# sailor-z/3DAHV

Measured on AMD Instinct MI355X. Metric: rotation hypotheses scored/sec (B=1), higher is better.
Workload: dtype f32; 1 GPU; CO3D pair (BASELINE.json configs[1]): B=1, ONE set of N_hyp=50000 Haar rotations split over the GPUs (contiguous shards, n_offset), source volume 16x8x8x8 (P=512 voxel sites x 16 ch), head 384->32->32, 64 positions; n_hyp_per_gpu=50000, n_hyp_total=50000, parallelism=hypothesis axis sharded x1, 8-byte key all-reduce(max), backend=single process, lanes=1

## Files before the change

### 3dahv_amd/_lib.py

```python
from __future__ import annotations

import ctypes
import os
import subprocess

_HERE = os.path.dirname(os.path.abspath(__file__))
CSRC = os.path.join(_HERE, "csrc")
LIB_PATH = os.path.join(CSRC, "libahv_hip.so")

AHV_SCORE_RESET_BEST = 1
AHV_SCORE_SPLIT_F16 = 2
AHV_SCORE_NO_TEAMS = 4
AHV_SCORE_SPARE_CUS_SHIFT = 8
AHV_SELECT_RESET_KEY = 1
AHV_KEY_EMPTY = -(1 << 63)
AHV_TOPK_MAX_K = 64
AHV_TOPK_RESET_LIST = 1
AHV_SO3_MAX_LADDER = 8
AHV_POSTERIOR_MAX_MODES = 16
AHV_POSTERIOR_RESET_STATE = 1
AHV_VIEWS_MAX = 16
AHV_VIEWS_RESET_BEST = 1
AHV_VIEWS_NO_ANGLE_LIMIT = 2

_vp = ctypes.c_void_p
_i64 = ctypes.c_int64
_int = ctypes.c_int
_u32 = ctypes.c_uint

SIGNATURES = {
    "ahv_abi_version": (_int, []),
    "ahv_last_error": (ctypes.c_char_p, []),
    "ahv_device_cu_count": (_int, []),
    "ahv_score_hypotheses_f32": (_int, [_vp, _vp, _vp, _i64, _i64, _vp, _vp, _vp, _int, _i64, _vp, _vp, _u32, _vp]),
    "ahv_score_hypotheses_clocked_f32": (_int, [_vp, _vp, _vp, _i64, _i64, _vp, _vp, _vp, _int, _i64, _vp, _vp, _u32,
                                                _vp, _vp]),
    "ahv_verify_pair_f32": (_int, [_vp, _vp, _vp, _i64, _i64, _vp, _vp, _vp, _int, _i64, _vp, _vp, _vp, _u32, _vp, _vp]),
    "ahv_unpack_best": (_int, [_vp, _int, _vp, _vp, _vp]),
    "ahv_reset_best": (_int, [_vp, _int, _vp]),
    "ahv_rotate_volume_f32": (_int, [_vp, _i64, _vp, _i64, _int, _int, _int, _int, _vp, _vp]),
    "ahv_rotate_volume_backward_f32": (_int, [_vp, _i64, _vp, _i64, _int, _int, _int, _int, _vp, _vp]),
    "ahv_forward_3d2d_f32": (_int, [_vp, _vp, _vp, _vp, _i64, _vp, _vp]),
    "ahv_score_features_f32": (_int, [_vp, _vp, _int, _i64, _vp, _vp]),
    "ahv_argmax_f32": (_int, [_vp, _int, _i64, _i64, _vp, _u32, _vp]),
    "ahv_random_rotations_f32": (_int, [ctypes.c_uint64, ctypes.c_uint64, _i64, _vp, _vp]),
    "ahv_so3_grid_f32": (_int, [_i64, _i64, _i64, _vp, _vp]),
    "ahv_select_rotation_f32": (_int, [_vp, _vp, _i64, _i64, _i64, _int, _vp, _vp, _vp, _u32, _vp]),
    "ahv_compose_rotations_f32": (_int, [_vp, _vp, _i64, _i64, _i64, _vp, _i64, _int, _vp, _vp]),
    "ahv_coarse_to_fine_f32": (_int, [_vp, _vp, _vp, _i64, _i64, _vp, _i64, _vp, _vp, _vp, _int, _vp, _vp, _vp, _vp, _vp,
                                      _vp, _vp, _vp, _vp, _vp, _u32, _vp]),
}

class BlockWeights(ctypes.Structure):
    _fields_ = [(n, _vp) for n in ("w_qkv", "w_out", "b_out", "ln1_g", "ln1_b", "w_ff1", "b_ff1", "w_ff2", "b_ff2",
                                   "ln2_g", "ln2_b")]


class AlignerWeights(ctypes.Structure):
    _fields_ = ([(n, _vp) for n in ("w_emb", "w_conv1", "w_conv2", "posemb", "gn_g", "gn_b")] +
                [("w_in", _vp * 2), ("b_in", _vp * 2), ("w_out", _vp * 2), ("b_out", _vp * 2),
                 ("w3d_1", _vp), ("w3d_2", _vp), ("blocks", ctypes.POINTER(BlockWeights)), ("depth", _int)])


SIGNATURES["ahv_forward_2d3d_workspace_bytes"] = (ctypes.c_size_t, [_int])
SIGNATURES["ahv_forward_2d3d_f32"] = (_int, [ctypes.POINTER(AlignerWeights), _vp, _vp, _int, _vp, ctypes.c_size_t, _vp,
                                             _vp, _vp])
SIGNATURES["ahv_score_hypotheses_backward_workspace_bytes"] = (ctypes.c_size_t, [_int, _i64])
SIGNATURES["ahv_score_hypotheses_backward_f32"] = (_int, [_vp, _vp, _vp, _i64, _vp, _vp, _vp, _int, _i64, _vp, _vp,
                                                          ctypes.c_size_t, _vp, _vp, _vp, _vp, _vp, _vp])
SIGNATURES["ahv_score_hypotheses_backward_saved_f32"] = SIGNATURES["ahv_score_hypotheses_backward_f32"]
SIGNATURES["ahv_score_hypotheses_train_f32"] = (_int, [_vp, _vp, _vp, _i64, _vp, _vp, _vp, _int, _i64, _vp, _vp, ctypes.c_size_t, _vp])
SIGNATURES["ahv_transformer_workspace_bytes"] = (ctypes.c_size_t, [_int])
SIGNATURES["ahv_transformer_blocks_f32"] = (_int, [ctypes.POINTER(BlockWeights), _int, _vp, _vp, _int, _vp,
                                                   ctypes.c_size_t, _vp])
SIGNATURES["ahv_topk_workspace_bytes"] = (ctypes.c_size_t, [_int, _i64, _int])
SIGNATURES["ahv_topk_f32"] = (_int, [_vp, _int, _i64, _i64, _int, _vp, _vp, ctypes.c_size_t, _u32, _vp])
SIGNATURES["ahv_topk_merge_keys"] = (_int, [_vp, _int, _int, _int, _vp, _u32, _vp])
SIGNATURES["ahv_select_topk_f32"] = (_int, [_vp, _int, _vp, _i64, _i64, _i64, _int, _vp, _vp, _vp, _u32, _vp])
SIGNATURES["ahv_compose_rotations_topk_f32"] = (_int, [_vp, _int, _vp, _i64, _i64, _i64, _vp, _i64, _int, _vp, _vp])
SIGNATURES["ahv_topk_modes_workspace_bytes"] = (ctypes.c_size_t, [_int, _i64, _int])
SIGNATURES["ahv_topk_modes_f32"] = (_int, [_vp, _vp, _i64, _int, _i64, _i64, _int, ctypes.c_float, _vp, _vp, ctypes.c_size_t, _vp])
SIGNATURES["ahv_score_rotation_grad_workspace_bytes"] = (ctypes.c_size_t, [_int, _i64])
SIGNATURES["ahv_score_rotation_grad_f32"] = (_int, [_vp, _vp, _vp, _i64, _vp, _vp, _vp, _int, _i64, _vp, _vp, ctypes.c_size_t,
                                                    _vp, _vp])
SIGNATURES["ahv_so3_ascent_candidates_f32"] = (_int, [_vp, _vp, _vp, _vp, _int, _int, _int, _vp, _vp])
SIGNATURES["ahv_so3_ascent_select_f32"] = (_int, [_vp, _vp, _vp, _int, _int, _int, _vp, _vp, _vp, _vp])
SIGNATURES["ahv_pose_posterior_state_bytes"] = (ctypes.c_size_t, [_int, _int])
SIGNATURES["ahv_pose_posterior_workspace_bytes"] = (ctypes.c_size_t, [_int, _i64, _int])
SIGNATURES["ahv_pose_posterior_f32"] = (_int, [_vp, _vp, _i64, _int, _i64, _vp, _int, ctypes.c_float, ctypes.c_float, _vp, _vp,
                                               ctypes.c_size_t, _u32, _vp])
SIGNATURES["ahv_pose_posterior_merge"] = (_int, [_vp, _int, _int, _int, ctypes.c_float, _vp, _u32, _vp])
SIGNATURES["ahv_pose_posterior_finish_f32"] = (_int, [_vp, _int, _int, ctypes.c_float] + [_vp] * 10 + [_vp])
SIGNATURES["ahv_view_rotations_f32"] = (_int, [_vp, _i64, _vp, _int, _int, _i64, _vp, _vp])
SIGNATURES["ahv_fuse_view_scores_f32"] = (_int, [_vp, _vp, _i64, _vp, _vp, _int, _int, _i64, _i64, ctypes.c_float, _vp, _vp, _u32,
                                                 _vp])

DIAG_SIGNATURES = {
    "ahv_score_hypotheses_clocked_f32": SIGNATURES.pop("ahv_score_hypotheses_clocked_f32"),
    "ahv_diag_score_plan": (_int, [_int, _i64, _u32, ctypes.POINTER(_int), ctypes.POINTER(_int), ctypes.POINTER(_i64)]),
}

_lib = None


class AhvError(RuntimeError):
    """A libahv_hip call returned a negative status."""


def build(force: bool = False) -> str:
    args = ["make", "-C", CSRC, "-j4"] + (["-B"] if force else [])
    proc = subprocess.run(args, stdout=subprocess.PIPE, stderr=subprocess.STDOUT, text=True)
    if proc.returncode != 0:
        raise RuntimeError("building libahv_hip.so failed:\n" + proc.stdout)
    return LIB_PATH


def load():
    global _lib
    if _lib is not None:
        return _lib
    import torch
    if not os.path.exists(LIB_PATH):
        raise ImportError(
            f"{LIB_PATH} not found: the HIP extension is required (no CPU fallback). "
            "Run `python -c 'import __graft_entry__ as g; g.build()'` or `make -C 3dahv_amd/csrc`."
        )
    lib = ctypes.CDLL(LIB_PATH)
    for name, (res, args) in list(SIGNATURES.items()) + list(DIAG_SIGNATURES.items()):
        fn = getattr(lib, name)
        fn.restype = res
        fn.argtypes = args
    _lib = lib
    return lib


def check(status: int, what: str) -> None:
    if status < 0:
        msg = load().ahv_last_error().decode("utf-8", "replace")
        raise AhvError(f"{what} failed with status {status}: {msg}")
```

### 3dahv_amd/csrc/ahv_abi.hip

```cpp
#include <hip/hip_runtime.h>

#include <cstdarg>
#include <cstdio>
#include <cstring>

#include "../../include/ahv.h"
#include "../../include/ahv_diag.h"
#include "ahv_launch.h"

namespace ahv {
hipError_t launch_unpack_best(const int64_t*, int, float*, int64_t*, hipStream_t);
hipError_t launch_rotate_volume(const float*, int64_t, const float*, int64_t, int, int, int, int, float*, int,
                                hipStream_t);
hipError_t launch_rotate_volume_backward(const float*, int64_t, const float*, int64_t, int, int, int, int, float*, int,
                                         hipStream_t);
hipError_t launch_forward_3d2d(const float*, const float*, const float*, const float*, int64_t, float*, int,
                               hipStream_t);
hipError_t launch_score_features(const float*, const float*, int, int64_t, float*, int, hipStream_t);
hipError_t launch_argmax(const float*, int, int64_t, int64_t, int64_t*, int, hipStream_t);
hipError_t launch_fill_keys(int64_t*, int, hipStream_t);
int topk_parts(int64_t N);
hipError_t launch_topk(const float*, int, int64_t, int64_t, int, int64_t*, int64_t*, bool, hipStream_t);
hipError_t launch_topk_merge(const int64_t*, int, int, int, int64_t*, bool, hipStream_t);
hipError_t launch_select_topk(int64_t*, int, const float*, int64_t, int64_t, int64_t, int, float*, float*, int64_t*, bool,
                              hipStream_t);
hipError_t launch_compose_rotations_topk(const int64_t*, int, const float*, int64_t, int64_t, int64_t, const float*, int64_t,
                                         int, float*, hipStream_t);
int64_t topk_modes_state_stride(int64_t N);
hipError_t launch_topk_modes(const float*, const float*, int64_t, int, int64_t, int64_t, int, float, int64_t*, int64_t*,
                             hipStream_t);
hipError_t launch_view_rotations(const float*, int64_t, const float*, int, int, int64_t, float*, hipStream_t);
hipError_t launch_fuse_views(const float*, const float*, int64_t, const float*, const float*, int, int, int64_t, int64_t, float,
                             bool, float*, int64_t*, hipStream_t);
size_t posterior_state_stride(int K);
int posterior_parts(int64_t N);
hipError_t launch_posterior(const float*, const float*, int64_t, int, int64_t, const float*, int, float, float, void*, void*, bool,
                            hipStream_t);
hipError_t launch_posterior_merge(const void*, int, int, int, float, void*, bool, hipStream_t);
hipError_t launch_posterior_finish(const void*, int, int, float, float*, float*, float*, int64_t*, float*, float*, float*, float*,
                                   float*, float*, hipStream_t);
hipError_t launch_random_rotations(uint64_t, uint64_t, int64_t, float*, hipStream_t);
hipError_t launch_so3_grid(int64_t, int64_t, int64_t, float*, hipStream_t);
hipError_t launch_score_backward(const float*, const float*, const float*, int64_t, const float*, const float*,
                                 const float*, int, int64_t, const float*, float*, float*, float*, float*, float*,
                                 float*, float*, int, hipStream_t, bool);
hipError_t launch_zero_fill(void* const* ptrs, const size_t* bytes, int count, hipStream_t stream);
hipError_t launch_score_rotation_grad(const float*, const float*, const float*, int64_t, const float*, const float*,
                                      const float*, int, int64_t, const float*, float*, float*, int, hipStream_t);
hipError_t launch_so3_ascent_candidates(const float*, const float*, const float*, const float*, int, int, int, float*,
                                        hipStream_t);
hipError_t launch_so3_ascent_select(const float*, const float*, const float*, int, int, int, float*, float*, float*,
                                    hipStream_t);
size_t transformer_workspace_floats(int B);
int transformer_blocks(const ahv_block_weights*, int, float*, float*, int, float*, hipStream_t, const char**);
size_t forward_2d3d_workspace_floats(int B);
int forward_2d3d(const ahv_aligner_weights*, const float*, const float*, int, float*, float*, float*, hipStream_t,
                 const char**);
}

namespace {

thread_local char g_err[256] = "";

int fail(int code, const char* fmt, ...)
{
    va_list ap;
    va_start(ap, fmt);
    vsnprintf(g_err, sizeof(g_err), fmt, ap);
    va_end(ap);
    return code;
}

int hip_fail(const char* what, hipError_t e)
{
    return fail(AHV_ELAUNCH, "%s: %s", what, hipGetErrorString(e));
}

int cu_count()
{
    static thread_local int cached_dev = -1, cached_cu = 0;
    int dev = 0;
    if (hipGetDevice(&dev) != hipSuccess) return -1;
    if (dev != cached_dev) {
        int cu = 0;
        if (hipDeviceGetAttribute(&cu, hipDeviceAttributeMultiprocessorCount, dev) != hipSuccess || cu <= 0)
            return -1;
        cached_dev = dev;
        cached_cu = cu;
    }
    return cached_cu;
}

}

extern "C" {

int ahv_abi_version(void) { return (2 << 16) | 3; }

const char* ahv_last_error(void) { return g_err; }

int ahv_device_cu_count(void)
{
    const int cu = cu_count();
    if (cu < 0) return fail(AHV_EDEVICE, "no usable HIP device");
    return cu;
}

static hipError_t zero_span(void* p, size_t bytes, hipStream_t s)
{
    void* const ptrs[1] = {p};
    const size_t n[1] = {bytes};
    return ahv::launch_zero_fill(ptrs, n, 1, s);
}

static int score_common(const char* who, const float* vol_src, const float* tgt, bool tgt_is_volume, const float* R,
                        int64_t r_batch_stride, int64_t n_offset, const float* W1, const float* W2, const float* b2, int B,
                        int64_t N, float* scores, int64_t* best_key, float* feat_tgt_out, unsigned flags,
                        uint64_t* clock_stamps, void* stream)
{
    if (B < 0 || N < 0) return fail(AHV_EINVAL, "%s: negative size (B=%d, N=%lld)", who, B, (long long)N);
    if (B > 0 && N > 0 && (!vol_src || !tgt || !R || !W1 || !W2 || !b2))
        return fail(AHV_EINVAL, "%s: null input pointer", who);
    if (r_batch_stride != 0 && r_batch_stride < N * 9)
        return fail(AHV_EINVAL, "%s: r_batch_stride %lld must be 0 or >= N*9", who, (long long)r_batch_stride);
    if (n_offset < 0 || n_offset + N > 4294967296ll)
        return fail(AHV_EINVAL, "%s: n_offset + N must fit in 32 bits", who);
    if (flags & ~(AHV_SCORE_RESET_BEST | AHV_SCORE_SPLIT_F16 | AHV_SCORE_NO_TEAMS | AHV_SCORE_SPARE_CUS_MASK))
        return fail(AHV_EINVAL, "%s: unknown flags 0x%x", who, flags);
    const bool split = (flags & AHV_SCORE_SPLIT_F16) != 0;
    hipStream_t s = static_cast<hipStream_t>(stream);
    if (best_key && (flags & AHV_SCORE_RESET_BEST) && B > 0) {
        hipError_t e = ahv::launch_fill_keys(best_key, B, s);
        if (e != hipSuccess) return hip_fail("score: key reset", e);
    }
    const int cu = cu_count();
    if (cu < 0) return fail(AHV_EDEVICE, "no usable HIP device");
    if (tgt_is_volume && split) {
        if (B > 0 && !feat_tgt_out)
            return fail(AHV_EINVAL, "%s: AHV_SCORE_SPLIT_F16 needs feat_tgt_out (the target features go through it)", who);
        if (B > 0) {
            hipError_t e = ahv::launch_forward_3d2d(tgt, W1, W2, b2, B, feat_tgt_out, cu, s);
            if (e != hipSuccess) return hip_fail("verify_pair: forward_3d2d launch", e);
        }
        tgt = feat_tgt_out;
        tgt_is_volume = false;
        feat_tgt_out = nullptr;
    }
    if (B == 0) return AHV_OK;
    if (N == 0 && !(tgt_is_volume && feat_tgt_out)) return AHV_OK;
    ahv::ScoreLaunch a;
    a.vol_src = vol_src; a.tgt = tgt; a.tgt_is_volume = tgt_is_volume; a.R = R;
    a.r_batch_stride = r_batch_stride; a.n_offset = n_offset; a.W1 = W1; a.W2 = W2; a.b2 = b2; a.B = B; a.N = N;
    a.scores = scores; a.best_key = best_key; a.feat_tgt_out = feat_tgt_out; a.num_cu = cu;
    a.spare_cu = (int)((flags & AHV_SCORE_SPARE_CUS_MASK) >> AHV_SCORE_SPARE_CUS_SHIFT);
    a.split_f16 = split; a.no_teams = (flags & AHV_SCORE_NO_TEAMS) != 0; a.clock_stamps = clock_stamps;
    hipError_t e = ahv::launch_score_hypotheses(a, s);
    if (e != hipSuccess) return hip_fail("score: launch", e);
    return AHV_OK;
}

int ahv_score_hypotheses_f32(const float* vol_src, const float* feat_tgt, const float* R,
                             int64_t r_batch_stride, int64_t n_offset, const float* W1, const float* W2,
                             const float* b2, int B, int64_t N, float* scores, int64_t* best_key,
                             unsigned flags, void* stream)
{
    return score_common("score", vol_src, feat_tgt, false, R, r_batch_stride, n_offset, W1, W2, b2, B, N, scores, best_key,
                        nullptr, flags, nullptr, stream);
}

int ahv_score_hypotheses_clocked_f32(const float* vol_src, const float* feat_tgt, const float* R,
                                     int64_t r_batch_stride, int64_t n_offset, const float* W1, const float* W2,
                                     const float* b2, int B, int64_t N, float* scores, int64_t* best_key,
                                     unsigned flags, uint64_t* clock_stamps, void* stream)
{
    if (!clock_stamps) return fail(AHV_EINVAL, "score_clocked: null clock_stamps");
    return score_common("score_clocked", vol_src, feat_tgt, false, R, r_batch_stride, n_offset, W1, W2, b2, B, N, scores,
                        best_key, nullptr, flags, clock_stamps, stream);
}

int ahv_diag_score_plan(int B, int64_t N, unsigned flags, int* gx, int* gy, int64_t* n_main)
{
    if (B < 1 || N < 0) return fail(AHV_EINVAL, "score_plan: bad shape (B=%d, N=%lld)", B, (long long)N);
    const int cu = cu_count();
    if (cu < 0) return fail(AHV_EDEVICE, "no usable HIP device");
    const bool teams = !(flags & AHV_SCORE_SPLIT_F16) && !(flags & AHV_SCORE_NO_TEAMS);
    const ahv::ScorePlan p = ahv::plan_score_launch(B, N, cu, (int)((flags & AHV_SCORE_SPARE_CUS_MASK) >> AHV_SCORE_SPARE_CUS_SHIFT), teams);
    if (gx) *gx = p.gx;
    if (gy) *gy = p.gy;
    if (n_main) *n_main = p.n_main;
    return AHV_OK;
}

int ahv_verify_pair_f32(const float* vol_src, const float* vol_tgt, const float* R, int64_t r_batch_stride,
                        int64_t n_offset, const float* W1, const float* W2, const float* b2, int B, int64_t N,
                        float* scores, int64_t* best_key, float* feat_tgt_out, unsigned flags, uint64_t* clock_stamps,
                        void* stream)
{
    return score_common("verify_pair", vol_src, vol_tgt, true, R, r_batch_stride, n_offset, W1, W2, b2, B, N, scores,
                        best_key, feat_tgt_out, flags, clock_stamps, stream);
}

int ahv_unpack_best(const int64_t* best_key, int B, float* best_score, int64_t* best_idx, void* stream)
{
    if (!best_key) return fail(AHV_EINVAL, "unpack: null best_key");
    if (B < 0) return fail(AHV_EINVAL, "unpack: negative B");
    if (B == 0) return AHV_OK;
    hipError_t e = ahv::launch_unpack_best(best_key, B, best_score, best_idx, static_cast<hipStream_t>(stream));
    if (e != hipSuccess) return hip_fail("unpack: launch", e);
    return AHV_OK;
}

int ahv_rotate_volume_f32(const float* vol, int64_t vol_batch_stride, const float* R, int64_t N, int C, int D,
                          int H, int W, float* out, void* stream)
{
    if (N < 0 || C < 1 || D < 1 || H < 1 || W < 1)
        return fail(AHV_EINVAL, "rotate_volume: bad shape N=%lld C=%d D=%d H=%d W=%d", (long long)N, C, D, H, W);
    if (vol_batch_stride < 0) return fail(AHV_EINVAL, "rotate_volume: negative batch stride");
    if (N == 0) return AHV_OK;
    if (!vol || !R || !out) return fail(AHV_EINVAL, "rotate_volume: null pointer");
    const int cu = cu_count();
    if (cu < 0) return fail(AHV_EDEVICE, "no usable HIP device");
    hipError_t e = ahv::launch_rotate_volume(vol, vol_batch_stride, R, N, C, D, H, W, out, cu,
                                             static_cast<hipStream_t>(stream));
    if (e != hipSuccess) return hip_fail("rotate_volume: launch", e);
    return AHV_OK;
}

int ahv_rotate_volume_backward_f32(const float* grad_out, int64_t vol_batch_stride, const float* R, int64_t N, int C,
                                   int D, int H, int W, float* grad_vol, void* stream)
{
    if (N < 0 || C < 1 || D < 1 || H < 1 || W < 1)
        return fail(AHV_EINVAL, "rotate_volume_backward: bad shape N=%lld C=%d D=%d H=%d W=%d", (long long)N, C, D, H, W);
    const int64_t vol_elems = (int64_t)C * D * H * W;
    if (vol_batch_stride != 0 && vol_batch_stride < vol_elems)
        return fail(AHV_EINVAL, "rotate_volume_backward: batch stride must be 0 or >= C*D*H*W");
    if (!grad_vol) return fail(AHV_EINVAL, "rotate_volume_backward: null grad_vol");
    hipStream_t s = static_cast<hipStream_t>(stream);
    const int64_t n_vol = vol_batch_stride == 0 ? 1 : N;
    if (n_vol > 0) {
        const size_t bytes = sizeof(float) * (size_t)(vol_batch_stride == 0 ? vol_elems : (N - 1) * vol_batch_stride + vol_elems);
        hipError_t e = zero_span(grad_vol, bytes, s);
        if (e != hipSuccess) return hip_fail("rotate_volume_backward: zero fill", e);
    }
    if (N == 0) return AHV_OK;
    if (!grad_out || !R) return fail(AHV_EINVAL, "rotate_volume_backward: null pointer");
    const int cu = cu_count();
    if (cu < 0) return fail(AHV_EDEVICE, "no usable HIP device");
    hipError_t e = ahv::launch_rotate_volume_backward(grad_out, vol_batch_stride, R, N, C, D, H, W, grad_vol, cu, s);
    if (e != hipSuccess) return hip_fail("rotate_volume_backward: launch", e);
    return AHV_OK;
}

int ahv_forward_3d2d_f32(const float* vol, const float* W1, const float* W2, const float* b2, int64_t M,
                         float* out, void* stream)
{
    if (M < 0) return fail(AHV_EINVAL, "forward_3d2d: negative M");
    if (M == 0) return AHV_OK;
    if (!vol || !W1 || !W2 || !b2 || !out) return fail(AHV_EINVAL, "forward_3d2d: null pointer");
    const int cu = cu_count();
    if (cu < 0) return fail(AHV_EDEVICE, "no usable HIP device");
    hipError_t e = ahv::launch_forward_3d2d(vol, W1, W2, b2, M, out, cu, static_cast<hipStream_t>(stream));
    if (e != hipSuccess) return hip_fail("forward_3d2d: launch", e);
    return AHV_OK;
}

int ahv_score_features_f32(const float* f_src, const float* f_tgt, int B, int64_t N, float* scores, void* stream)
{
    if (B < 0 || N < 0) return fail(AHV_EINVAL, "score_features: negative size");
    if (B == 0 || N == 0) return AHV_OK;
    if (!f_src || !f_tgt || !scores) return fail(AHV_EINVAL, "score_features: null pointer");
    const int cu = cu_count();
    if (cu < 0) return fail(AHV_EDEVICE, "no usable HIP device");
    hipError_t e = ahv::launch_score_features(f_src, f_tgt, B, N, scores, cu, static_cast<hipStream_t>(stream));
    if (e != hipSuccess) return hip_fail("score_features: launch", e);
    return AHV_OK;
}

int ahv_compose_rotations_f32(const int64_t* best_key, const float* R, int64_t r_batch_stride, int64_t n_offset,
                                 int64_t N, const float* D, int64_t N2, int B, float* out, void* stream)
{
    if (B < 0 || N < 0 || N2 < 0) return fail(AHV_EINVAL, "compose_rotations: negative size");
    if (B == 0 || N2 == 0) return AHV_OK;
    if (!best_key || !R || !D || !out) return fail(AHV_EINVAL, "compose_rotations: null pointer");
    if (N == 0) return fail(AHV_EINVAL, "compose_rotations: empty rotation set");
    if (r_batch_stride != 0 && r_batch_stride < N * 9) return fail(AHV_EINVAL, "compose_rotations: bad r_batch_stride");
    hipError_t e = ahv::launch_compose_rotations_topk(best_key, 1, R, r_batch_stride, n_offset, N, D, N2, B, out,
                                                      static_cast<hipStream_t>(stream));
    if (e != hipSuccess) return hip_fail("compose_rotations: launch", e);
    return AHV_OK;
}

int ahv_coarse_to_fine_f32(const float* vol_src, const float* vol_tgt, const float* R, int64_t r_batch_stride, int64_t N,
                           const float* D, int64_t N2, const float* W1, const float* W2, const float* b2, int B,
                           float* scores_coarse, float* scores_fine, int64_t* keys, uint32_t* sync, float* feat_tgt_out,
                           float* R_pred, float* fine_score, int64_t* fine_idx, float* coarse_score, int64_t* coarse_idx,
                           unsigned flags, void* stream)
{
    if (B < 0 || N < 0 || N2 < 0) return fail(AHV_EINVAL, "coarse_to_fine: negative size (B=%d, N=%lld, N2=%lld)", B, (long long)N, (long long)N2);
    if (B == 0) return AHV_OK;
    if (N == 0 || N2 == 0) return fail(AHV_EINVAL, "coarse_to_fine: empty hypothesis set (N=%lld, N2=%lld)", (long long)N, (long long)N2);
    if (!vol_src || !vol_tgt || !R || !D || !W1 || !W2 || !b2) return fail(AHV_EINVAL, "coarse_to_fine: null input pointer");
    if (!keys || !sync) return fail(AHV_EINVAL, "coarse_to_fine: keys and sync are required (2 B keys, 2 B + 1 counters)");
    if (r_batch_stride != 0 && r_batch_stride < N * 9)
        return fail(AHV_EINVAL, "coarse_to_fine: r_batch_stride %lld must be 0 or >= N*9", (long long)r_batch_stride);
    if (N > 4294967296ll || N2 > 4294967296ll) return fail(AHV_EINVAL, "coarse_to_fine: indices must fit in 32 bits");
    if (flags & ~(AHV_SCORE_NO_TEAMS | AHV_SCORE_SPARE_CUS_MASK)) return fail(AHV_EINVAL, "coarse_to_fine: unknown flags 0x%x", flags);
    const int cu = cu_count();
    if (cu < 0) return fail(AHV_EDEVICE, "no usable HIP device");
    ahv::CoarseToFineLaunch a;
    ahv::ScoreLaunch& c = a.coarse;
    c.vol_src = vol_src; c.tgt = vol_tgt; c.tgt_is_volume = true; c.R = R; c.r_batch_stride = r_batch_stride; c.n_offset = 0;
    c.W1 = W1; c.W2 = W2; c.b2 = b2; c.B = B; c.N = N; c.scores = scores_coarse; c.best_key = keys;
    c.feat_tgt_out = feat_tgt_out; c.num_cu = cu;
    c.spare_cu = (int)((flags & AHV_SCORE_SPARE_CUS_MASK) >> AHV_SCORE_SPARE_CUS_SHIFT);
    c.split_f16 = false; c.no_teams = (flags & AHV_SCORE_NO_TEAMS) != 0; c.clock_stamps = nullptr;
    a.D = D; a.N2 = N2; a.scores2 = scores_fine; a.best_key2 = keys + B; a.sync = sync; a.R_pred = R_pred;
    a.fine_score = fine_score; a.coarse_score = coarse_score; a.fine_idx = fine_idx; a.coarse_idx = coarse_idx;
    hipError_t e = ahv::launch_coarse_to_fine(a, static_cast<hipStream_t>(stream));
    if (e != hipSuccess) return hip_fail("coarse_to_fine: launch", e);
    return AHV_OK;
}

int ahv_reset_best(int64_t* best_key, int B, void* stream)
{
    if (B < 0) return fail(AHV_EINVAL, "reset_best: negative B");
    if (B == 0) return AHV_OK;
    if (!best_key) return fail(AHV_EINVAL, "reset_best: null best_key");
    hipError_t e = ahv::launch_fill_keys(best_key, B, static_cast<hipStream_t>(stream));
    if (e != hipSuccess) return hip_fail("reset_best: launch", e);
    return AHV_OK;
}

int ahv_select_rotation_f32(int64_t* best_key, const float* R, int64_t r_batch_stride, int64_t n_offset, int64_t N,
                            int B, float* R_out, float* best_score, int64_t* best_idx, unsigned flags, void* stream)
{
    if (B < 0 || N < 0) return fail(AHV_EINVAL, "select_rotation: negative size");
    if (flags & ~AHV_SELECT_RESET_KEY) return fail(AHV_EINVAL, "select_rotation: unknown flags 0x%x", flags);
    if (B == 0) return AHV_OK;
    if (!best_key) return fail(AHV_EINVAL, "select_rotation: null best_key");
    if (R_out && (!R || N == 0)) return fail(AHV_EINVAL, "select_rotation: R_out needs a rotation set");
    if (r_batch_stride != 0 && r_batch_stride < N * 9) return fail(AHV_EINVAL, "select_rotation: bad r_batch_stride");
    hipError_t e = ahv::launch_select_topk(best_key, 1, R, r_batch_stride, n_offset, N, B, R_out, best_score, best_idx,
                                           (flags & AHV_SELECT_RESET_KEY) != 0, static_cast<hipStream_t>(stream));
    if (e != hipSuccess) return hip_fail("select_rotation: launch", e);
    return AHV_OK;
}

size_t ahv_transformer_workspace_bytes(int B) { return sizeof(float) * ahv::transformer_workspace_floats(B); }

int ahv_transformer_blocks_f32(const ahv_block_weights* blocks, int depth, float* x_src, float* x_tgt, int B,
                               void* workspace, size_t workspace_bytes, void* stream)
{
    if (depth < 0 || B < 0) return fail(AHV_EINVAL, "transformer_blocks: negative size");
    if (depth == 0 || B == 0) return AHV_OK;
    if (!blocks || !x_src || !x_tgt || !workspace) return fail(AHV_EINVAL, "transformer_blocks: null pointer");
    if (workspace_bytes < ahv_transformer_workspace_bytes(B))
        return fail(AHV_EINVAL, "transformer_blocks: workspace of %zu bytes, need %zu", workspace_bytes,
                    ahv_transformer_workspace_bytes(B));
    if ((reinterpret_cast<uintptr_t>(workspace) & 15) || (reinterpret_cast<uintptr_t>(x_src) & 15) ||
        (reinterpret_cast<uintptr_t>(x_tgt) & 15))
        return fail(AHV_EINVAL, "transformer_blocks: buffers must be 16-byte aligned");
    for (int i = 0; i < 4 * depth; ++i) {
        const ahv_block_weights& w = blocks[i];
        if (!w.w_qkv || !w.w_out || !w.b_out || !w.ln1_g || !w.ln1_b || !w.w_ff1 || !w.b_ff1 || !w.w_ff2 || !w.b_ff2 ||
            !w.ln2_g || !w.ln2_b)
            return fail(AHV_EINVAL, "transformer_blocks: null weight pointer in block %d", i);
    }
    const char* what = "";
    const int rc = ahv::transformer_blocks(blocks, depth, x_src, x_tgt, B, static_cast<float*>(workspace),
                                           static_cast<hipStream_t>(stream), &what);
    if (rc != 0) return fail(AHV_ELAUNCH, "transformer_blocks: %s: %s", what, hipGetErrorString((hipError_t)rc));
    return AHV_OK;
}

size_t ahv_forward_2d3d_workspace_bytes(int B) { return sizeof(float) * ahv::forward_2d3d_workspace_floats(B); }

int ahv_forward_2d3d_f32(const ahv_aligner_weights* w, const float* layer4_src, const float* layer4_tgt, int B,
                         void* workspace, size_t workspace_bytes, float* vol_src, float* vol_tgt, void* stream)
{
    if (B < 0) return fail(AHV_EINVAL, "forward_2d3d: negative B");
    if (B == 0) return AHV_OK;
    if (!w || !layer4_src || !layer4_tgt || !workspace || !vol_src || !vol_tgt)
        return fail(AHV_EINVAL, "forward_2d3d: null pointer");
    if (!w->w_emb || !w->w_conv1 || !w->w_conv2 || !w->posemb || !w->gn_g || !w->gn_b || !w->w_in[0] || !w->w_in[1] ||
        !w->b_in[0] || !w->b_in[1] || !w->w_out[0] || !w->w_out[1] || !w->b_out[0] || !w->b_out[1] || !w->w3d_1 ||
        !w->w3d_2 || (w->depth > 0 && !w->blocks))
        return fail(AHV_EINVAL, "forward_2d3d: null weight pointer");
    if (w->depth < 0) return fail(AHV_EINVAL, "forward_2d3d: negative depth");
    if (workspace_bytes < ahv_forward_2d3d_workspace_bytes(B))
        return fail(AHV_EINVAL, "forward_2d3d: workspace of %zu bytes, need %zu", workspace_bytes,
                    ahv_forward_2d3d_workspace_bytes(B));
    if (reinterpret_cast<uintptr_t>(workspace) & 15) return fail(AHV_EINVAL, "forward_2d3d: workspace must be 16-byte aligned");
    const char* what = "";
    const int rc = ahv::forward_2d3d(w, layer4_src, layer4_tgt, B, static_cast<float*>(workspace), vol_src, vol_tgt,
                                     static_cast<hipStream_t>(stream), &what);
    if (rc != 0) return fail(AHV_ELAUNCH, "forward_2d3d: %s: %s", what, hipGetErrorString((hipError_t)rc));
    return AHV_OK;
}

size_t ahv_score_hypotheses_backward_workspace_bytes(int B, int64_t N)
{
    if (B <= 0 || N <= 0) return 0;
    const int cu = cu_count();
    const size_t wgs = cu > 0 ? (size_t)cu : 1024;
    return sizeof(float) * (2048 * (size_t)B * (size_t)N + (((size_t)B + 3) & ~(size_t)3) + wgs * 32 * 384);
}

static int score_backward_common(const float* vol_src, const float* feat_tgt, const float* R,
                                 int64_t r_batch_stride, const float* W1, const float* W2, const float* b2,
                                 int B, int64_t N, const float* grad_scores, void* workspace,
                                 size_t workspace_bytes, float* grad_vol_src, float* grad_feat_tgt,
                                 float* grad_W1, float* grad_W2, float* grad_b2, void* stream, bool saved_u);

int ahv_score_hypotheses_backward_f32(const float* vol_src, const float* feat_tgt, const float* R,
                                      int64_t r_batch_stride, const float* W1, const float* W2, const float* b2,
                                      int B, int64_t N, const float* grad_scores, void* workspace,
                                      size_t workspace_bytes, float* grad_vol_src, float* grad_feat_tgt,
                                      float* grad_W1, float* grad_W2, float* grad_b2, void* stream)
{
    return score_backward_common(vol_src, feat_tgt, R, r_batch_stride, W1, W2, b2, B, N, grad_scores, workspace, workspace_bytes,
                                 grad_vol_src, grad_feat_tgt, grad_W1, grad_W2, grad_b2, stream, false);
}

int ahv_score_hypotheses_backward_saved_f32(const float* vol_src, const float* feat_tgt, const float* R,
                                            int64_t r_batch_stride, const float* W1, const float* W2, const float* b2,
                                            int B, int64_t N, const float* grad_scores, void* workspace,
                                            size_t workspace_bytes, float* grad_vol_src, float* grad_feat_tgt,
                                            float* grad_W1, float* grad_W2, float* grad_b2, void* stream)
{
    return score_backward_common(vol_src, feat_tgt, R, r_batch_stride, W1, W2, b2, B, N, grad_scores, workspace, workspace_bytes,
                                 grad_vol_src, grad_feat_tgt, grad_W1, grad_W2, grad_b2, stream, true);
}

int ahv_score_hypotheses_train_f32(const float* vol_src, const float* feat_tgt, const float* R, int64_t r_batch_stride,
                                   const float* W1, const float* W2, const float* b2, int B, int64_t N, float* scores,
                                   void* workspace, size_t workspace_bytes, void* stream)
{
    if (B < 0 || N < 0) return fail(AHV_EINVAL, "score_train: negative size");
    if (B > 65535) return fail(AHV_EINVAL, "score_train: B > 65535");
    if (B == 0 || N == 0) return AHV_OK;
    if (!vol_src || !feat_tgt || !R || !W1 || !W2 || !b2 || !scores || !workspace) return fail(AHV_EINVAL, "score_train: null pointer");
    if (r_batch_stride != 0 && r_batch_stride != N * 9) return fail(AHV_EINVAL, "score_train: r_batch_stride must be 0 or N*9");
    if (workspace_bytes < ahv_score_hypotheses_backward_workspace_bytes(B, N))
        return fail(AHV_EINVAL, "score_train: workspace of %zu bytes, need %zu (ahv_score_hypotheses_backward_workspace_bytes)",
                    workspace_bytes, ahv_score_hypotheses_backward_workspace_bytes(B, N));
    if (reinterpret_cast<uintptr_t>(workspace) & 15) return fail(AHV_EINVAL, "score_train: workspace must be 16-byte aligned");
    const int cu = cu_count();
    if (cu <= 0) return fail(AHV_EDEVICE, "score_train: no usable HIP device");
    ahv::ScoreLaunch a{};
    a.vol_src = vol_src; a.tgt = feat_tgt; a.tgt_is_volume = false; a.R = R; a.r_batch_stride = r_batch_stride; a.n_offset = 0;
    a.W1 = W1; a.W2 = W2; a.b2 = b2; a.B = B; a.N = N; a.scores = scores; a.best_key = nullptr; a.feat_tgt_out = nullptr;
    a.num_cu = cu; a.spare_cu = 0; a.split_f16 = false; a.no_teams = true; a.clock_stamps = nullptr;
    hipError_t e = ahv::launch_score_hypotheses_train(a, static_cast<float*>(workspace), static_cast<hipStream_t>(stream));
    if (e != hipSuccess) return hip_fail("score_train: launch", e);
    return AHV_OK;
}

static int score_backward_common(const float* vol_src, const float* feat_tgt, const float* R,
                                 int64_t r_batch_stride, const float* W1, const float* W2, const float* b2,
                                 int B, int64_t N, const float* grad_scores, void* workspace,
                                 size_t workspace_bytes, float* grad_vol_src, float* grad_feat_tgt,
                                 float* grad_W1, float* grad_W2, float* grad_b2, void* stream, bool saved_u)
{
    if (B < 0 || N < 0) return fail(AHV_EINVAL, "score_backward: negative size");
    if (B > 65535) return fail(AHV_EINVAL, "score_backward: B > 65535");
    if (!grad_W1 || !grad_W2 || !grad_b2) return fail(AHV_EINVAL, "score_backward: null weight-gradient pointer");
    if (B > 0 && (!grad_vol_src || !grad_feat_tgt)) return fail(AHV_EINVAL, "score_backward: null gradient pointer");
    if (B > 0 && N > 0) {
        if (!vol_src || !feat_tgt || !R || !W1 || !W2 || !b2 || !grad_scores || !workspace)
            return fail(AHV_EINVAL, "score_backward: null pointer");
        if (r_batch_stride != 0 && r_batch_stride != N * 9)
            return fail(AHV_EINVAL, "score_backward: r_batch_stride must be 0 or N*9");
        if (workspace_bytes < ahv_score_hypotheses_backward_workspace_bytes(B, N))
            return fail(AHV_EINVAL, "score_backward: workspace of %zu bytes, need %zu", workspace_bytes,
                        ahv_score_hypotheses_backward_workspace_bytes(B, N));
        if (reinterpret_cast<uintptr_t>(workspace) & 15)
            return fail(AHV_EINVAL, "score_backward: workspace must be 16-byte aligned");
    }
    const int cu = cu_count();
    if (cu <= 0) return fail(AHV_EDEVICE, "score_backward: no usable HIP device");
    hipError_t e = ahv::launch_score_backward(vol_src, feat_tgt, R, r_batch_stride, W1, W2, b2, B, N, grad_scores,
                                              static_cast<float*>(workspace),
                                              static_cast<float*>(workspace) + 2048 * (size_t)B * (size_t)N + (((size_t)B + 3) & ~(size_t)3),
                                              grad_vol_src, grad_feat_tgt, grad_W1, grad_W2, grad_b2, cu,
                                              static_cast<hipStream_t>(stream), saved_u);
    if (e != hipSuccess) return hip_fail("score_backward: launch", e);
    return AHV_OK;
}

int ahv_random_rotations_f32(uint64_t seed, uint64_t offset, int64_t N, float* out, void* stream)
{
    if (N < 0) return fail(AHV_EINVAL, "random_rotations: negative N");
    if (N == 0) return AHV_OK;
    if (!out) return fail(AHV_EINVAL, "random_rotations: null pointer");
    hipError_t e = ahv::launch_random_rotations(seed, offset, N, out, static_cast<hipStream_t>(stream));
    if (e != hipSuccess) return hip_fail("random_rotations: launch", e);
    return AHV_OK;
}

int ahv_so3_grid_f32(int64_t n_total, int64_t offset, int64_t N, float* out, void* stream)
{
    if (N < 0 || offset < 0 || n_total <= 0 || offset + N > n_total)
// ... 361 lines not shown
```

### 3dahv_amd/csrc/ahv_launch.h

```cpp
#pragma once
#include <hip/hip_runtime.h>
#include <stdint.h>

namespace ahv {

struct ScoreLaunch {
    const float* vol_src;
    const float* tgt;
    bool tgt_is_volume;
    const float* R;
    int64_t r_batch_stride, n_offset;
    const float *W1, *W2, *b2;
    int B;
    int64_t N;
    float* scores;
    int64_t* best_key;
    float* feat_tgt_out;
    int num_cu, spare_cu;
    bool split_f16;
    bool no_teams;
    uint64_t* clock_stamps;
};

struct ScorePlan {
    int gx, gy;
    int64_t n_main;
};

ScorePlan plan_score_launch(int B, int64_t N, int num_cu, int spare_cu, bool teams);
hipError_t launch_score_hypotheses(const ScoreLaunch& a, hipStream_t stream);
hipError_t launch_score_hypotheses_train(const ScoreLaunch& a, float* u_out, hipStream_t stream);

struct CoarseToFineLaunch {
    ScoreLaunch coarse;
    const float* D;
    int64_t N2;
    float* scores2;
    int64_t* best_key2;
    uint32_t* sync;
    float* R_pred;
    float *fine_score, *coarse_score;
    int64_t *fine_idx, *coarse_idx;
};
hipError_t launch_coarse_to_fine(const CoarseToFineLaunch& a, hipStream_t stream);

}
```

### 3dahv_amd/csrc/ahv_score.hip

```cpp
#define AHV_FP32_LOW_HALF
#include "ahv_dual.h"
#include "ahv_split.h"
#include "ahv_team.h"
#include "ahv_exact.h"
#include "ahv_launch.h"

namespace ahv {

__device__ __forceinline__ int opaque(int x)
{
    asm volatile("" : "+v"(x));
    return x;
}

__device__ __forceinline__ float swap_add32(float a, float b)
{
    const auto r = __builtin_amdgcn_permlane32_swap(__float_as_uint(a), __float_as_uint(b), false, false);
    return __uint_as_float(r[0]) + __uint_as_float(r[1]);
}

__device__ __forceinline__ float swap_add16(float a, float b)
{
    const auto r = __builtin_amdgcn_permlane16_swap(__float_as_uint(a), __float_as_uint(b), false, false);
    return __uint_as_float(r[0]) + __uint_as_float(r[1]);
}

template <bool XDL>
__device__ __forceinline__ void hyp_tile_sums(float& ss, float& dt, const f32x4& v0, const f32x4& v1, const f32x4& g0, const f32x4& g1)
{
    f32x2 s2 = {0.0f, 0.0f}, d2 = {0.0f, 0.0f};
#pragma unroll
    for (int m2 = 0; m2 < 2; ++m2)
#pragma unroll
        for (int hh = 0; hh < 2; ++hh) {
            const f32x4& vv = m2 ? v1 : v0;
            const f32x4& gg = m2 ? g1 : g0;
            const f32x2 x = {vv[2 * hh], vv[2 * hh + 1]};
            const f32x2 g = {gg[2 * hh], gg[2 * hh + 1]};
            s2 = __builtin_elementwise_fma(x, x, s2);
            d2 = __builtin_elementwise_fma(x, g, d2);
        }
    ss = s2[0] + (XDL ? low_half(s2[1]) : s2[1]);
    dt = d2[0] + (XDL ? low_half(d2[1]) : d2[1]);
}

__device__ __forceinline__ float hyp_score_tail(const float (&ss)[4], const float (&dt)[4])
{
#pragma clang fp contract(off)
    float s2[2], d2[2];
#pragma unroll
    for (int i = 0; i < 2; ++i) {
        s2[i] = swap_add32(ss[i], ss[2 + i]);
        d2[i] = swap_add32(dt[i], dt[2 + i]);
    }
    const float s1 = swap_add16(s2[0], s2[1]);
    const float d1 = swap_add16(d2[0], d2[1]);
    const float c = d1 * __builtin_amdgcn_rsqf(fmaxf(s1, 1e-24f));
    const float tot = wave_sum_dpp(c);
    return __builtin_bit_cast(float, __builtin_amdgcn_readlane(__builtin_bit_cast(int, tot), 63)) * (1.0f / 64.0f);
}

template <bool XDL>
__device__ __forceinline__ float hyp_score_rs(const f32x4 (&v)[2][4], const f32x4 (&tg)[4][2], int lane)
{
    float ss[4], dt[4];
#pragma unroll
    for (int t = 0; t < 4; ++t) hyp_tile_sums<XDL>(ss[t], dt[t], v[0][t], v[1][t], tg[t][0], tg[t][1]);
    return hyp_score_tail(ss, dt);
}

template <bool XDL>
__device__ __forceinline__ float team_tile_score(const f32x4 (&v)[2], const f32x4& g0, const f32x4& g1, int lane)
{
#pragma clang fp contract(off)
    float ss, dt;
    hyp_tile_sums<XDL>(ss, dt, v[0], v[1], g0, g1);
    ss += __shfl_xor(ss, 32, 64);
    dt += __shfl_xor(dt, 32, 64);
    ss += __shfl_xor(ss, 16, 64);
    dt += __shfl_xor(dt, 16, 64);
    const float c = lane < 16 ? dt * __builtin_amdgcn_rsqf(fmaxf(ss, 1e-24f)) : 0.0f;
    return wave_sum_dpp(c);
}

__device__ __forceinline__ void team_gather(float* buf, const float* srcT, const GatherHyp& gh, const GatherDst& gdst, int member,
                                            unsigned* done_ctr, unsigned done_target)
{
    HatState st;
    if (member < 2) {
        hat_prologue_rt(st, srcT, gh, (float)member);
        team_wait(done_ctr, done_target);
        hat_body(st, buf, gdst);
    } else {
        const float qf = (float)(3 - member);
        hat_voxel_rt(st.vx[0], srcT, gh, 0, qf);
        hat_voxel_rt(st.vx[1], srcT, gh, 1, qf);
        hat_prologue_mirror(st, srcT);
        team_wait(done_ctr, done_target);
        hat_body<true>(st, buf, gdst);
    }
}

#ifdef AHV_STAMPS
__device__ unsigned long long g_stamps[2048 * 16];
__device__ unsigned long long g_wgstamps[1024 * 4];
__device__ unsigned long long g_wgclk[1024 * 2];
#define AHV_STAMP(var)                                                                 \
    __builtin_amdgcn_sched_barrier(0);                                                 \
    asm volatile("s_memtime %0\n\ts_waitcnt lgkmcnt(0)" : "=s"(var)::"memory");        \
    __builtin_amdgcn_sched_barrier(0);
#else
#define AHV_STAMP(var)
#endif

constexpr int kDualThreads = 512;

struct C2fArgs {
    const float* D;
    long N2, n_main2;
    key_t* best_key2;
    float* scores2;
    unsigned* sync;
    float* R_pred;
    float *fine_score, *coarse_score;
    long *fine_idx, *coarse_idx;
};
constexpr unsigned kC2fSpinLimit = 1u << 20;

struct ExactCompose {
    float r[9];
    bool on;
};

struct NoCompose {
    static constexpr bool on = false;
    static constexpr float r[9] = {0.f, 0.f, 0.f, 0.f, 0.f, 0.f, 0.f, 0.f, 0.f};
};

template <bool SPLIT, typename Compose>
__device__ __attribute__((noinline)) key_t score_share_exact(const float* lds_src, const float* lds_w1, float* buf, const float* W1,
                                                             const float* W2, const float* b2, const float* Rb, Compose Rstar,
                                                             long N, long h0, long hstep, float* scores_b, long n_offset, key_t best,
                                                             int lane)
{
    const int rl = lane < 9 ? lane : 8;
    DualFrags f;
    load_dual_frags(f, W2, b2, lane);
    for (long he = h0; he < N; he += hstep) {
        const float Re = Rb[he * 9 + rl];
        float Rm[9];
#pragma unroll
        for (int i = 0; i < 9; ++i) Rm[i] = __builtin_bit_cast(float, __builtin_amdgcn_readlane(__builtin_bit_cast(int, Re), i));
        if (Rstar.on) {
            float d[9];
#pragma unroll
            for (int i = 0; i < 9; ++i) d[i] = Rm[i];
#pragma unroll
            for (int a = 0; a < 3; ++a)
#pragma unroll
                for (int c = 0; c < 3; ++c)
                    Rm[a * 3 + c] = Rstar.r[a * 3] * d[c] + Rstar.r[a * 3 + 1] * d[3 + c] + Rstar.r[a * 3 + 2] * d[6 + c];
        }
        f32x4 acc[2][4];
        if constexpr (SPLIT) exact_hypothesis_gemm1(acc, buf, lds_src, Rm, W1FragsGlobal{W1, lane}, lane);
        else exact_hypothesis_gemm1(acc, buf, lds_src, Rm, W1FragsLds{reinterpret_cast<const f32x4*>(lds_w1) + lane}, lane);
        f32x4 v[2][4];
        gemm2_dual_exact(v, acc, f);
        f32x4 tg[4][2];
#pragma unroll
        for (int t = 0; t < 4; ++t)
#pragma unroll
            for (int m2 = 0; m2 < 2; ++m2)
                tg[t][m2] = *reinterpret_cast<const f32x4*>(lds_src + ((2 * t + m2) * 64 + lane) * kSrcStride + 16);
        const float s = hyp_score_rs<SPLIT || kFp32LowHalf>(v, tg, lane);
        if (scores_b != nullptr && lane == 0) scores_b[he] = s;
        const key_t key = pack_key(s, (unsigned)(n_offset + he));
        best = key > best ? key : best;
    }
    return best;
}

template <bool SPLIT, bool TGT, bool C2F, bool SAVE_U = false>
__device__ __forceinline__ void score_hypotheses_body(
    const float* __restrict__ vol_src, const float* __restrict__ tgt, const float* __restrict__ R,
    long r_batch_stride, long n_offset, const float* __restrict__ W1, const float* __restrict__ W2,
    const float* __restrict__ b2, int B, long N, long n_main, float* __restrict__ scores,
    key_t* __restrict__ best_key, float* __restrict__ feat_tgt_out, unsigned long long* __restrict__ clk, const C2fArgs& cf)
{
    static_assert(!(SPLIT && TGT), "the split-f16 kernel takes ready-made target features");
    static_assert(!C2F || (TGT && !SPLIT), "the two-stage launch is the fp32 verify kernel");
    static_assert(!SAVE_U || (!SPLIT && !TGT && !C2F), "u is saved by the fp32 scorer with ready-made target features");
    if constexpr (!SPLIT) asm volatile("" ::: "v255");
    __shared__ __attribute__((aligned(1024))) float lds_src[kSrcFloats];
    __shared__ __attribute__((aligned(16))) float lds_w1[kW1TableFloats];
    __shared__ __attribute__((aligned(16))) float lds_q[8 * kQuarterFloats];
    __shared__ TeamSync lds_team;
    __shared__ NonFinite lds_nf;
    __shared__ unsigned long long lds_t_entry[2];
    if (clk != nullptr && threadIdx.x == 0) {
        lds_t_entry[0] = __builtin_amdgcn_s_memrealtime();
        lds_t_entry[1] = __builtin_amdgcn_s_memtime();
    }
    const int tid = threadIdx.x;
    const int lane = tid & 63;
    const int wave = __builtin_amdgcn_readfirstlane(tid >> 6);
    const float* srcT = lds_src;
    float* buf = lds_q + wave * kQuarterFloats;

    static_assert(kSplitTableBytes == sizeof(float) * kW1TableFloats && kSplitImageBytes == sizeof(float) * kQuarterFloats, "LDS budget");

#ifdef AHV_STAMPS
    const unsigned long long wg_t_entry = __builtin_amdgcn_s_memrealtime();
    unsigned long long wg_t_loop = 0;
#endif
    if (!SPLIT && tid < (int)(sizeof(TeamSync) / 4)) reinterpret_cast<unsigned*>(&lds_team)[tid] = 0u;
    if (tid < (int)(sizeof(NonFinite) / 4)) reinterpret_cast<unsigned*>(&lds_nf)[tid] = 0u;
    SrcRegs sv;
    TgtRegs tv;
    W1Regs w1r;
    const bool w1_rows = (reinterpret_cast<unsigned long long>(W1) & 15ull) == 0;
    if (!SPLIT) {
        if (w1_rows) w1_regs_load(w1r, W1, tid);
        src_regs_load(sv, vol_src + (long)blockIdx.y * (16 * 512), tid);
        tgt_regs_load<TGT>(tv, tgt, (int)blockIdx.y, tid);
    }
    int w1_exp = 0, w2_exp = 0;
    if (SPLIT) {
        float m = 0.0f;
        bool bad = non_finite(W2[tid]) || non_finite(W2[tid + 512]) || non_finite(b2[tid & 31]);
        for (int i = tid; i < 32 * 384; i += kDualThreads) {
            m = fmaxf(m, fabsf(W1[i]));
            bad = bad || non_finite(W1[i]);
        }
        w1_exp = split_prescale_exp(block_absmax(m, lds_q, tid));
        if (bad) lds_nf.weights = 1u;
        stage_w1_split(reinterpret_cast<f16x8*>(lds_w1), W1, ldexpf(1.0f, w1_exp), tid, kDualThreads);
        w2_exp = split_prescale_exp(block_absmax(fmaxf(fabsf(W2[tid]), fabsf(W2[tid + 512])), lds_q, tid));
    }
    DualFrags f0;
    bool w_bad = false;
    if (!SPLIT) {
        load_dual_frags(f0, W2, b2, lane);
        bool bad = false;
        if (w1_rows) {
            w1_regs_store(lds_w1, w1r, tid);
#pragma unroll
            for (int k = 0; k < 6; ++k)
#pragma unroll
                for (int e = 0; e < 4; ++e) bad = bad || non_finite(w1r.w[k][e]);
        } else {
            stage_w1_table(lds_w1, W1, tid, kDualThreads);
            for (int i = tid; i < 32 * 384; i += kDualThreads) bad = bad || non_finite(W1[i]);
        }
#pragma unroll
        for (int i = 0; i < 16; ++i) bad = bad || non_finite((&f0.a2[0][0][0])[i]);
#pragma unroll
        for (int i = 0; i < 8; ++i) bad = bad || non_finite(f0.bias[i >> 2][i & 3]);
        w_bad = bad;
    }
    const int team = wave >> 2, member = wave & 3;
    unsigned team_rounds = 0;
    unsigned samples_done = 0;
    const GatherLane glane = gather_lane(lane);
    const GatherDst gdst = gather_dst_swizzled(lane);
    const SplitDst sdst = split_dst(lane);
    SplitResident w1res;
    if (SPLIT) {
        __syncthreads();
        split_load_resident(w1res, reinterpret_cast<const f16x8*>(lds_w1), lane);
    }
    const long hstep = (long)gridDim.x * 8;

    for (int b = blockIdx.y; b < B; b += gridDim.y) {
        __syncthreads();
        const int lane_s = opaque(lane), tid_s = wave * 64 + lane_s;
        const unsigned gen = samples_done + 1u;
        if (w_bad) lds_nf.weights = 1u;
        DualFrags f = f0;
        Split2Frags w2s;
        int exp_sum = 0;
        if (SPLIT) {
            load_dual_frags(f, W2, b2, lane_s);
            split_w2_frags(w2s, f, ldexpf(1.0f, w2_exp));
            bool bad;
            exp_sum = w2_exp + w1_exp + stage_src_volume_scaled(lds_src, vol_src + (long)b * (16 * 512), lds_q, tid_s, bad);
            if (bad) lds_nf.src_gen = gen;
        } else {
            src_regs_store(lds_src, sv, tid_s);
            bool bad = false;
#pragma unroll
            for (int c = 0; c < 16; ++c) bad = bad || non_finite(sv.x[c]);
            if (bad) lds_nf.src_gen = gen;
            if constexpr (TGT) {
                bool tbad = false;
#pragma unroll
                for (int c = 0; c < 16; ++c) tbad = tbad || non_finite(tv.q[c].x) || non_finite(tv.q[c].y);
                if (tbad) lds_nf.tgt_gen = gen;
            }
            tgt_regs_store<TGT>(lds_src, buf, tv, tid_s);
        }
        if (SPLIT) {
            const float* ft = tgt + (long)b * (32 * 64);
            const int l = tid_s & 63, t = tid_s >> 7, m2 = (tid_s >> 6) & 1;
            f32x4 x;
#pragma unroll
            for (int r = 0; r < 4; ++r) x[r] = ft[(16 * m2 + 4 * (l >> 4) + r) * 64 + 16 * t + (l & 15)];
            *reinterpret_cast<f32x4*>(lds_src + tid_s * kSrcStride + 16) = x;
        }
        __syncthreads();
        const bool nf_w = __builtin_amdgcn_readfirstlane((int)lds_nf.weights) != 0;
#ifdef AHV_DIAG_NO_EXACT
        const bool exact = false;
#else
        const bool exact = nf_w || (unsigned)__builtin_amdgcn_readfirstlane((int)lds_nf.src_gen) == gen;
#endif
        if constexpr (SPLIT) {
            if (nf_w) {
                restage_src_volume_unscaled(lds_src, vol_src + (long)b * (16 * 512), wave * 64 + opaque(lane));
                __syncthreads();
            }
        }
        bool tg_ready = !TGT;
        if constexpr (TGT) {
            if (team == 1) {
                f32x4 u[2], v[2];
                team_round(u, lds_w1, lds_q + 4 * kQuarterFloats, lds_team, 1, member, team_rounds, lane_s);
                ++team_rounds;
                if (nf_w || (unsigned)__builtin_amdgcn_readfirstlane((int)lds_nf.tgt_gen) == gen) team_head_exact(v, u, f0);
                else team_head(v, u, f0);
                const float inv = 1.0f / fmaxf(sqrtf(team_sumsq(v)), 1e-12f);
#pragma unroll
                for (int m2 = 0; m2 < 2; ++m2) {
                    const f32x4 x = v[m2] * inv;
                    *reinterpret_cast<f32x4*>(lds_src + ((2 * member + m2) * 64 + lane_s) * kSrcStride + 16) = x;
                    if (feat_tgt_out != nullptr && blockIdx.x == 0) {
                        const int ol = lane_s;
#pragma unroll
                        for (int r = 0; r < 4; ++r)
                            feat_tgt_out[(long)b * (32 * 64) + (16 * m2 + 4 * (ol >> 4) + r) * 64 + 16 * member + (ol & 15)] = x[r];
                    }
                }
                team_signal(&lds_team.tgt_ready, lane_s);
                team_wait(&lds_team.done[1], 4u * team_rounds);
            }
        }
        auto tg_wait = [&]() {
            if (TGT && !tg_ready) {
                team_wait(&lds_team.tgt_ready, 4u * (samples_done + 1u));
                tg_ready = true;
            }
        };
#ifdef AHV_STAMPS
        wg_t_loop = __builtin_amdgcn_s_memrealtime();
        const unsigned long long wg_c_loop = __builtin_amdgcn_s_memtime();
#endif
        const float* Rb0 = R + (long)b * r_batch_stride;
        const int residue = xcd_residue(blockIdx.x, gridDim.x, gridDim.y);
        float Rstar[9] = {0.f, 0.f, 0.f, 0.f, 0.f, 0.f, 0.f, 0.f, 0.f};
        auto hyp_rotation = [&](float (&Rm)[9], bool compose) {
            if (C2F && compose) {
                float d[9];
#pragma unroll
                for (int i = 0; i < 9; ++i) d[i] = Rm[i];
#pragma unroll
                for (int a = 0; a < 3; ++a)
#pragma unroll
                    for (int c = 0; c < 3; ++c)
                        Rm[a * 3 + c] = Rstar[a * 3] * d[c] + Rstar[a * 3 + 1] * d[3 + c] + Rstar[a * 3 + 2] * d[6 + c];
            }
        };
      for (int stage = 0; stage < (C2F ? 2 : 1); ++stage) {
        const bool st1 = C2F && stage != 0;
        const float* Rb = st1 ? cf.D : Rb0;
        const long N_s = st1 ? cf.N2 : N, n_main_s = st1 ? cf.n_main2 : n_main, n_offset_s = st1 ? 0l : n_offset;
        float* scores_s = st1 ? cf.scores2 : scores;
        key_t* key_s = st1 ? cf.best_key2 : best_key;
        if (st1) {
            __syncthreads();
            if (tid == 0) {
                __hip_atomic_fetch_add(cf.sync + 2 * b, 1u, __ATOMIC_RELEASE, __HIP_MEMORY_SCOPE_AGENT);
                unsigned polls = 0;
                while (__hip_atomic_load(cf.sync + 2 * b, __ATOMIC_ACQUIRE, __HIP_MEMORY_SCOPE_AGENT) < gridDim.x) {
                    __builtin_amdgcn_s_sleep(16);
                    if (++polls > kC2fSpinLimit) {
                        __hip_atomic_fetch_or(cf.sync + 2 * B, 1u, __ATOMIC_RELAXED, __HIP_MEMORY_SCOPE_AGENT);
                        break;
                    }
                }
            }
            __syncthreads();
            const key_t kc = __hip_atomic_load(best_key + b, __ATOMIC_RELAXED, __HIP_MEMORY_SCOPE_AGENT);
            long idx = key_index(kc) - n_offset;
            idx = (kc == kKeyEmpty || idx < 0 || idx >= N) ? 0 : idx;
#pragma unroll
            for (int i = 0; i < 9; ++i)
                Rstar[i] = __builtin_bit_cast(float, __builtin_amdgcn_readfirstlane(__builtin_bit_cast(int, Rb0[idx * 9 + i])));
        }
        key_t best = kKeyEmpty;
        const int rl = lane < 9 ? lane : 8;
        auto score_remainder_by_teams = [&]() {
            const long tstep = 2l * gridDim.x;
            long ht = n_main_s + (long)team * gridDim.x + residue;
            if (ht < N_s) {
                long h_prev = -1;
                float Rt = Rb[ht * 9 + rl];
                auto team_emit = [&]() {
                    const float* pp = lds_team.part[team][(team_rounds + 1u) & 1u];
                    const float sc = ((pp[3] + pp[2]) + (pp[1] + pp[0])) * (1.0f / 64.0f);
                    if (scores_s != nullptr && lane == 0) scores_s[(long)b * N_s + h_prev] = sc;
                    const key_t key = pack_key(sc, (unsigned)(n_offset_s + h_prev));
                    best = key > best ? key : best;
                };
                for (; ht < N_s; ht += tstep) {
                    float Rm[9];
#pragma unroll
                    for (int i = 0; i < 9; ++i) Rm[i] = __builtin_bit_cast(float, __builtin_amdgcn_readlane(__builtin_bit_cast(int, Rt), i));
                    hyp_rotation(Rm, st1);
                    if (ht + tstep < N_s) Rt = Rb[(ht + tstep) * 9 + rl];
                    GatherHyp gh;
                    gather_hyp(gh, Rm, glane);
                    team_gather(buf, srcT, gh, gdst, member, &lds_team.done[team], 4u * team_rounds);
                    wave_lds_fence();
                    f32x4 u[2], v[2];
                    team_round(u, lds_w1, lds_q + 4 * team * kQuarterFloats, lds_team, team, member, team_rounds, lane);
                    if (member == 0 && h_prev >= 0) team_emit();
                    tg_wait();
                    team_head(v, u, f);
                    const f32x4 g0 = *reinterpret_cast<const f32x4*>(lds_src + ((2 * member) * 64 + lane) * kSrcStride + 16);
                    const f32x4 g1 = *reinterpret_cast<const f32x4*>(lds_src + ((2 * member + 1) * 64 + lane) * kSrcStride + 16);
                    const float tot = team_tile_score<kFp32LowHalf>(v, g0, g1, lane);
                    if (lane == 63) lds_team.part[team][team_rounds & 1u][member] = tot;
                    ++team_rounds;
                    h_prev = ht;
                }
                team_signal(&lds_team.arrive[team], lane);
                team_wait(&lds_team.arrive[team], 4u * (team_rounds + 1u));
                if (member == 0) team_emit();
                team_signal(&lds_team.done[team], lane);
                ++team_rounds;
                team_wait(&lds_team.done[team], 4u * team_rounds);
            }
        };
        if (exact) {
            if constexpr (TGT) tg_wait();
            const long h0 = (long)wave * gridDim.x + residue;
            float* sc_b = scores_s != nullptr ? scores_s + (long)b * N_s : nullptr;
            if constexpr (C2F) {
                ExactCompose ec;
#pragma unroll
                for (int i = 0; i < 9; ++i) ec.r[i] = Rstar[i];
                ec.on = st1;
                best = score_share_exact<SPLIT>(lds_src, lds_w1, buf, W1, W2, b2, Rb, ec, N_s, h0, hstep, sc_b, n_offset_s, best, lane);
            } else {
                best = score_share_exact<SPLIT>(lds_src, lds_w1, buf, W1, W2, b2, Rb, NoCompose{}, N_s, h0, hstep, sc_b, n_offset_s, best, lane);
            }
            if constexpr (SPLIT) split_load_resident(w1res, reinterpret_cast<const f16x8*>(lds_w1), lane);
            if constexpr (SAVE_U) {
                const f32x4 qn = f32x4{__builtin_nanf(""), __builtin_nanf(""), __builtin_nanf(""), __builtin_nanf("")};
                for (long he = h0; he < N_s; he += hstep) {
                    float* uo = feat_tgt_out + ((long)b * N_s + he) * 2048 + lane * 4;
#pragma unroll
                    for (int i = 0; i < 8; ++i) *reinterpret_cast<f32x4*>(uo + i * 256) = qn;
                }
            }
        } else {
        if constexpr (!SPLIT && !SAVE_U) score_remainder_by_teams();
        long h = (long)wave * gridDim.x + residue;
        float Rn = h < n_main_s ? Rb[h * 9 + rl] : 0.0f;
#ifdef AHV_STAMPS
        unsigned long long tsum[11] = {0, 0, 0, 0, 0, 0, 0, 0, 0, 0, 0};
#endif
        for (; h < n_main_s; h += hstep) {
            float Rm[9];
#pragma unroll
            for (int i = 0; i < 9; ++i) Rm[i] = __builtin_bit_cast(float, __builtin_amdgcn_readlane(__builtin_bit_cast(int, Rn), i));
            hyp_rotation(Rm, st1);
            {
                const long hn = (h + hstep < n_main_s) ? h + hstep : h;
                Rn = Rb[hn * 9 + rl];
            }
            f32x4 acc[2][4];
#pragma unroll
            for (int m = 0; m < 2; ++m)
#pragma unroll
                for (int t = 0; t < 4; ++t) acc[m][t] = f32x4{0.f, 0.f, 0.f, 0.f};

#ifdef AHV_STAMPS
            unsigned long long ts[11];
#define AHV_TS(i) AHV_STAMP(ts[i])
#else
#define AHV_TS(i)
#endif
            AHV_TS(0)
            if constexpr (SPLIT) {
                char* cbuf = reinterpret_cast<char*>(buf);
                const f16x8* w1s = reinterpret_cast<const f16x8*>(lds_w1);
                GatherHyp gh;
                gather_hyp(gh, Rm, glane);
                HatState st;
                hat_prologue<0, true, kSplitHatDepth>(st, srcT, gh);
                hat_body_split(st, cbuf, sdst); wave_lds_fence(); AHV_TS(1)
                gemm1_quarter_split<0>(acc, w1res, w1s, cbuf, lane, [] {}); wave_lds_fence(); AHV_TS(2)
                hat_prologue_mirror<kSplitHatDepth>(st, srcT);
                hat_body_split<true>(st, cbuf, sdst); wave_lds_fence(); AHV_TS(3)
                gemm1_quarter_split<3>(acc, w1res, w1s, cbuf, lane, [] {}); wave_lds_fence(); AHV_TS(4)
                hat_prologue<1, true, kSplitHatDepth>(st, srcT, gh);
                hat_body_split(st, cbuf, sdst); wave_lds_fence(); AHV_TS(5)
                gemm1_quarter_split<1>(acc, w1res, w1s, cbuf, lane, [] {}); wave_lds_fence(); AHV_TS(6)
                hat_prologue_mirror<kSplitHatDepth>(st, srcT);
                hat_body_split<true>(st, cbuf, sdst); wave_lds_fence(); AHV_TS(7)
                gemm1_quarter_split<2>(acc, w1res, w1s, cbuf, lane, [] {}); wave_lds_fence(); AHV_TS(8)
            } else {
                GatherHyp gh;
                gather_hyp(gh, Rm, glane);
                HatState st;
                hat_prologue<0>(st, srcT, gh);
                hat_body(st, buf, gdst); wave_lds_fence(); AHV_TS(1)
                gemm1_quarter_pipe<0>(acc, lds_w1, buf, lane, [&] { hat_prologue_mirror(st, srcT); }); wave_lds_fence(); AHV_TS(2)
                hat_body<true>(st, buf, gdst); wave_lds_fence(); AHV_TS(3)
                gemm1_quarter_pipe<3>(acc, lds_w1, buf, lane, [&] { hat_prologue<1>(st, srcT, gh); }); wave_lds_fence(); AHV_TS(4)
                hat_body(st, buf, gdst); wave_lds_fence(); AHV_TS(5)
                gemm1_quarter_pipe<1>(acc, lds_w1, buf, lane, [&] { hat_prologue_mirror(st, srcT); }); wave_lds_fence(); AHV_TS(6)
                hat_body<true>(st, buf, gdst); wave_lds_fence(); AHV_TS(7)
                gemm1_quarter_pipe<2>(acc, lds_w1, buf, lane, [] {}); wave_lds_fence(); AHV_TS(8)
            }

            tg_wait();
            float s;
            if constexpr (SPLIT) {
                const Gemm2Scale sc = gemm2_split_scale(acc, exp_sum);
                float ss[4], dt[4];
#pragma unroll
                for (int t = 0; t < 4; ++t) {
                    const f32x4 g0 = *reinterpret_cast<const f32x4*>(lds_src + ((2 * t) * 64 + lane) * kSrcStride + 16);
                    const f32x4 g1 = *reinterpret_cast<const f32x4*>(lds_src + ((2 * t + 1) * 64 + lane) * kSrcStride + 16);
                    f32x4 v0, v1;
                    gemm2_split_tile(v0, v1, acc[0][t], acc[1][t], w2s, f.bias, sc);
                    hyp_tile_sums<true>(ss[t], dt[t], v0, v1, g0, g1);
                }
                AHV_TS(9)
                s = hyp_score_tail(ss, dt);
            } else {
                if constexpr (SAVE_U) {
                    float* uo = feat_tgt_out + ((long)b * N_s + h) * 2048 + lane * 4;
#pragma unroll
                    for (int m = 0; m < 2; ++m)
#pragma unroll
                        for (int t = 0; t < 4; ++t) *reinterpret_cast<f32x4*>(uo + (t * 2 + m) * 256) = acc[m][t];
                }
                f32x4 v[2][4];
                gemm2_dual(v, acc, f);
                AHV_TS(9)
                f32x4 tg[4][2];
#pragma unroll
                for (int t = 0; t < 4; ++t)
#pragma unroll
                    for (int m2 = 0; m2 < 2; ++m2)
                        tg[t][m2] = *reinterpret_cast<const f32x4*>(lds_src + ((2 * t + m2) * 64 + lane) * kSrcStride + 16);
                s = hyp_score_rs<kFp32LowHalf>(v, tg, lane);
            }
            if (scores_s != nullptr && lane == 0) scores_s[(long)b * N_s + h] = s;
            const key_t key = pack_key(s, (unsigned)(n_offset_s + h));
            best = key > best ? key : best;
            AHV_TS(10)
#ifdef AHV_STAMPS
            for (int i = 0; i < 10; ++i) tsum[i] += ts[i + 1] - ts[i];
            tsum[10] += 1;
#endif
        }
#ifdef AHV_STAMPS
        if (lane == 0) {
            const int gw = (blockIdx.x * 8 + wave) & 2047;
            for (int i = 0; i < 11; ++i) g_stamps[gw * 16 + i] = tsum[i];
        }
#endif
        }
        if (key_s != nullptr && lane == 0 && best != kKeyEmpty) atomicMax(key_s + b, best);
      }
        ++samples_done;
        if (!SPLIT) {
            const int bn = b + (int)gridDim.y < B ? b + (int)gridDim.y : b;
            const int tid_e = wave * 64 + opaque(lane);
            src_regs_load(sv, vol_src + (long)bn * (16 * 512), tid_e);
            tgt_regs_load<TGT>(tv, tgt, bn, tid_e);
        }
        if constexpr (C2F) {
            __syncthreads();
            if (tid == 0) {
                const unsigned before = __hip_atomic_fetch_add(cf.sync + 2 * b + 1, 1u, __ATOMIC_ACQ_REL, __HIP_MEMORY_SCOPE_AGENT);
                if (before == gridDim.x - 1) {
                    const key_t kc = __hip_atomic_load(best_key + b, __ATOMIC_RELAXED, __HIP_MEMORY_SCOPE_AGENT);
                    const key_t kf = __hip_atomic_load(cf.best_key2 + b, __ATOMIC_RELAXED, __HIP_MEMORY_SCOPE_AGENT);
                    const bool gave_up = __hip_atomic_load(cf.sync + 2 * B, __ATOMIC_RELAXED, __HIP_MEMORY_SCOPE_AGENT) != 0u;
                    const float nanv = __builtin_nanf("");
                    if (cf.coarse_score) cf.coarse_score[b] = gave_up ? nanv : (kc == kKeyEmpty) ? -INFINITY : key_score(kc);
                    if (cf.coarse_idx) cf.coarse_idx[b] = (gave_up || kc == kKeyEmpty) ? -1l : key_index(kc);
                    if (cf.fine_score) cf.fine_score[b] = gave_up ? nanv : (kf == kKeyEmpty) ? -INFINITY : key_score(kf);
                    const long fi = (gave_up || kf == kKeyEmpty) ? -1l : key_index(kf);
                    if (cf.fine_idx) cf.fine_idx[b] = fi;
                    if (cf.R_pred) {
                        float Rm[9];
#pragma unroll
                        for (int i = 0; i < 9; ++i) Rm[i] = (fi >= 0 && fi < cf.N2) ? cf.D[fi * 9 + i] : (gave_up ? nanv : 0.0f);
                        if (fi >= 0 && fi < cf.N2) hyp_rotation(Rm, true);
#pragma unroll
                        for (int i = 0; i < 9; ++i) cf.R_pred[b * 9 + i] = Rm[i];
                    }
                    __hip_atomic_store(best_key + b, kKeyEmpty, __ATOMIC_RELAXED, __HIP_MEMORY_SCOPE_AGENT);
                    __hip_atomic_store(cf.best_key2 + b, kKeyEmpty, __ATOMIC_RELAXED, __HIP_MEMORY_SCOPE_AGENT);
                    __hip_atomic_store(cf.sync + 2 * b, 0u, __ATOMIC_RELAXED, __HIP_MEMORY_SCOPE_AGENT);
                    __hip_atomic_store(cf.sync + 2 * b + 1, 0u, __ATOMIC_RELAXED, __HIP_MEMORY_SCOPE_AGENT);
                }
            }
        }
#ifdef AHV_STAMPS
        __syncthreads();
        if (tid == 0) {
            unsigned long long* o = g_wgstamps + 4 * (blockIdx.x & 1023);
            o[0] = wg_t_entry;
            o[1] = wg_t_loop;
            o[2] = __builtin_amdgcn_s_memrealtime();
            o[3] = __builtin_amdgcn_s_getreg(((4 - 1) << 11) | 20);
            g_wgclk[2 * (blockIdx.x & 1023)] = wg_c_loop;
            g_wgclk[2 * (blockIdx.x & 1023) + 1] = __builtin_amdgcn_s_memtime();
        }
#endif
    }
    if (clk != nullptr) {
        __syncthreads();
        if (wave == 0 && lane == 0) {
            unsigned long long* o = clk + 4 * (blockIdx.y * gridDim.x + blockIdx.x);
            o[0] = lds_t_entry[1];
            o[1] = lds_t_entry[0];
            o[2] = __builtin_amdgcn_s_memtime();
            o[3] = __builtin_amdgcn_s_memrealtime();
        }
    }
}

template <bool SPLIT, bool TGT>
__global__ __launch_bounds__(kDualThreads, 2) void score_hypotheses_dual_kernel(
    const float* __restrict__ vol_src, const float* __restrict__ tgt, const float* __restrict__ R,
    long r_batch_stride, long n_offset, const float* __restrict__ W1, const float* __restrict__ W2,
    const float* __restrict__ b2, int B, long N, long n_main, float* __restrict__ scores,
    key_t* __restrict__ best_key, float* __restrict__ feat_tgt_out, unsigned long long* __restrict__ clk)
{
    score_hypotheses_body<SPLIT, TGT, false>(vol_src, tgt, R, r_batch_stride, n_offset, W1, W2, b2, B, N, n_main, scores, best_key,
                                             feat_tgt_out, clk, C2fArgs{});
}

__global__ __launch_bounds__(kDualThreads, 2) void score_hypotheses_train_kernel(
    const float* __restrict__ vol_src, const float* __restrict__ tgt, const float* __restrict__ R,
    long r_batch_stride, const float* __restrict__ W1, const float* __restrict__ W2,
    const float* __restrict__ b2, int B, long N, float* __restrict__ scores, float* __restrict__ u_out)
{
    score_hypotheses_body<false, false, false, true>(vol_src, tgt, R, r_batch_stride, 0l, W1, W2, b2, B, N, N, scores, nullptr, u_out,
                                                     nullptr, C2fArgs{});
}

__global__ __launch_bounds__(kDualThreads, 2) void coarse_to_fine_kernel(
    const float* __restrict__ vol_src, const float* __restrict__ tgt, const float* __restrict__ R,
    long r_batch_stride, long n_offset, const float* __restrict__ W1, const float* __restrict__ W2,
    const float* __restrict__ b2, int B, long N, long n_main, float* __restrict__ scores,
    key_t* __restrict__ best_key, float* __restrict__ feat_tgt_out, C2fArgs cf)
{
    score_hypotheses_body<false, true, true>(vol_src, tgt, R, r_batch_stride, n_offset, W1, W2, b2, B, N, n_main, scores, best_key,
                                             feat_tgt_out, nullptr, cf);
}

__global__ void unpack_best_kernel(const key_t* __restrict__ best_key, int B, float* __restrict__ best_score,
                                   long* __restrict__ best_idx)
{
    const int b = blockIdx.x * blockDim.x + threadIdx.x;
    if (b >= B) return;
    const key_t k = best_key[b];
    if (best_score) best_score[b] = (k == kKeyEmpty) ? -INFINITY : key_score(k);
    if (best_idx) best_idx[b] = (k == kKeyEmpty) ? -1l : key_index(k);
}

}

namespace ahv {

ScorePlan plan_score_launch(int B, int64_t N, int num_cu, int spare_cu, bool teams)
{
    ScorePlan p;
    int avail = num_cu - spare_cu;
    if (avail < 1) avail = 1;
    p.gy = B < avail ? B : avail;
    if (p.gy < 1) p.gy = 1;
    int64_t gx = avail / p.gy;
    const int64_t want = teams ? (N + 1) / 2 : (N + 3) / 4;
    if (gx > want) gx = want;
    if (gx < 1) gx = 1;
    p.gx = (int)gx;
    const int64_t slots = 8 * gx, full = N / slots, rem = N - full * slots;
    p.n_main = (teams && rem > 0 && rem <= 2 * gx) ? full * slots : N;
    return p;
}

hipError_t launch_score_hypotheses(const ScoreLaunch& a, hipStream_t stream)
{
    static_assert(sizeof(key_t) == sizeof(int64_t), "key width");
    const bool teams = !a.split_f16 && !a.no_teams;
    const ScorePlan p = plan_score_launch(a.B, a.N, a.num_cu, a.spare_cu, teams);
    const dim3 grid(p.gx, p.gy), block(kDualThreads);
    auto* key = reinterpret_cast<key_t*>(a.best_key);
    auto* clk = reinterpret_cast<unsigned long long*>(a.clock_stamps);
    if (a.split_f16) {
        if (a.tgt_is_volume) return hipErrorInvalidValue;
        hipLaunchKernelGGL((score_hypotheses_dual_kernel<true, false>), grid, block, 0, stream, a.vol_src, a.tgt, a.R,
                           (long)a.r_batch_stride, (long)a.n_offset, a.W1, a.W2, a.b2, a.B, (long)a.N, (long)p.n_main, a.scores,
                           key, a.feat_tgt_out, clk);
    } else if (a.tgt_is_volume) {
        hipLaunchKernelGGL((score_hypotheses_dual_kernel<false, true>), grid, block, 0, stream, a.vol_src, a.tgt, a.R,
                           (long)a.r_batch_stride, (long)a.n_offset, a.W1, a.W2, a.b2, a.B, (long)a.N, (long)p.n_main, a.scores,
                           key, a.feat_tgt_out, clk);
    } else {
        hipLaunchKernelGGL((score_hypotheses_dual_kernel<false, false>), grid, block, 0, stream, a.vol_src, a.tgt, a.R,
                           (long)a.r_batch_stride, (long)a.n_offset, a.W1, a.W2, a.b2, a.B, (long)a.N, (long)p.n_main, a.scores,
                           key, a.feat_tgt_out, clk);
    }
    return hipGetLastError();
}

hipError_t launch_score_hypotheses_train(const ScoreLaunch& a, float* u_out, hipStream_t stream)
{
    if (a.split_f16 || a.tgt_is_volume || a.scores == nullptr || u_out == nullptr) return hipErrorInvalidValue;
    const ScorePlan p = plan_score_launch(a.B, a.N, a.num_cu, a.spare_cu, false);
    hipLaunchKernelGGL(score_hypotheses_train_kernel, dim3(p.gx, p.gy), dim3(kDualThreads), 0, stream, a.vol_src, a.tgt, a.R,
                       (long)a.r_batch_stride, a.W1, a.W2, a.b2, a.B, (long)a.N, a.scores, u_out);
    return hipGetLastError();
}

hipError_t launch_coarse_to_fine(const CoarseToFineLaunch& a, hipStream_t stream)
{
    const ScoreLaunch& c = a.coarse;
    const bool teams = !c.no_teams;
    const ScorePlan p = plan_score_launch(c.B, c.N, c.num_cu, c.spare_cu, teams);
    const int64_t slots = 8 * (int64_t)p.gx, full2 = a.N2 / slots, rem2 = a.N2 - full2 * slots;
    const int64_t n_main2 = (teams && rem2 > 0 && rem2 <= 2 * (int64_t)p.gx) ? full2 * slots : a.N2;
    if ((int64_t)p.gx * p.gy > c.num_cu) return hipErrorInvalidConfiguration;
    C2fArgs cf;
    cf.D = a.D;
    cf.N2 = (long)a.N2;
    cf.n_main2 = (long)n_main2;
    cf.best_key2 = reinterpret_cast<key_t*>(a.best_key2);
    cf.scores2 = a.scores2;
    cf.sync = a.sync;
    cf.R_pred = a.R_pred;
    cf.fine_score = a.fine_score;
    cf.coarse_score = a.coarse_score;
    cf.fine_idx = reinterpret_cast<long*>(a.fine_idx);
    cf.coarse_idx = reinterpret_cast<long*>(a.coarse_idx);
    hipLaunchKernelGGL(coarse_to_fine_kernel, dim3(p.gx, p.gy), dim3(kDualThreads), 0, stream, c.vol_src, c.tgt, c.R,
                       (long)c.r_batch_stride, (long)c.n_offset, c.W1, c.W2, c.b2, c.B, (long)c.N, (long)p.n_main, c.scores,
                       reinterpret_cast<key_t*>(c.best_key), c.feat_tgt_out, cf);
    return hipGetLastError();
}

hipError_t launch_unpack_best(const int64_t* best_key, int B, float* best_score, int64_t* best_idx,
                              hipStream_t stream)
{
    const int threads = 64;
    hipLaunchKernelGGL(unpack_best_kernel, dim3((B + threads - 1) / threads), dim3(threads), 0, stream,
                       reinterpret_cast<const key_t*>(best_key), B, best_score, reinterpret_cast<long*>(best_idx));
    return hipGetLastError();
}

}
```

### 3dahv_amd/csrc/ahv_team.h

```cpp
#pragma once
#include "ahv_dual.h"

namespace ahv {

struct TeamSync {
    unsigned arrive[2];
    unsigned done[2];
    unsigned tgt_ready;
    float part[2][2][4];
};

__device__ __forceinline__ void team_signal(unsigned* ctr, int lane)
{
    __builtin_amdgcn_s_waitcnt(0xc07f);
    asm volatile("" ::: "memory");
    if (lane == 0) __hip_atomic_fetch_add(ctr, 1u, __ATOMIC_RELAXED, __HIP_MEMORY_SCOPE_WORKGROUP);
    asm volatile("" ::: "memory");
}

__device__ __forceinline__ void team_wait(unsigned* ctr, unsigned target)
{
    while ((int)(__hip_atomic_load(ctr, __ATOMIC_RELAXED, __HIP_MEMORY_SCOPE_WORKGROUP) - target) < 0) __builtin_amdgcn_s_sleep(1);
    asm volatile("" ::: "memory");
    __builtin_amdgcn_wave_barrier();
}

struct TeamZ {
    f32x4 a[4];
    float b[8];
};

__device__ __forceinline__ void team_z_load(TeamZ& z, const f32x4* T, const float* bufs, int Q, int zoff)
{
    const f32x4* Tz = T + (32 + 4 * Q) * 64;
    const float* img = bufs + Q * kQuarterFloats + zoff;
#pragma unroll
    for (int cpp = 0; cpp < 4; ++cpp) {
        z.a[cpp] = Tz[cpp * 64];
#pragma unroll
        for (int ci = 0; ci < 2; ++ci) z.b[2 * cpp + ci] = img[2 * (2 * cpp + ci) * 128];
    }
}

__device__ __forceinline__ void team_z_mfma(f32x4 (&u)[2], const TeamZ& z)
{
#pragma unroll
    for (int cpp = 0; cpp < 4; ++cpp)
#pragma unroll
        for (int ci = 0; ci < 2; ++ci) {
            u[0] = __builtin_amdgcn_mfma_f32_16x16x4f32(z.a[cpp][2 * ci + 0], z.b[2 * cpp + ci], u[0], 0, 0, 0);
            u[1] = __builtin_amdgcn_mfma_f32_16x16x4f32(z.a[cpp][2 * ci + 1], z.b[2 * cpp + ci], u[1], 0, 0, 0);
        }
}

template <int K>
__device__ __forceinline__ void g1_load_xy(G1Chunk& ck, const f32x4* T, const float* buf, int i0, int j, int kq)
{
    static_assert(K < 8, "x and y slabs");
    const int c0 = 4 * (K & 3);
#pragma unroll
    for (int i = 0; i < 4; ++i) {
        const int c = c0 + i;
        ck.a[i] = T[((K < 4 ? 0 : 16) + c) * 64];
#pragma unroll
        for (int hh = 0; hh < 2; ++hh)
            ck.b[2 * i + hh] = (K < 4) ? buf[c * 128 + qoff(i0, j, 4 * hh + kq)]
                                       : buf[c * 128 + qoff(i0, 4 * hh + kq, j)];
    }
}

__device__ __forceinline__ void g1_mfma_xy(f32x4 (&u)[2], const G1Chunk& ck)
{
#pragma unroll
    for (int i = 0; i < 4; ++i)
#pragma unroll
        for (int hh = 0; hh < 2; ++hh) {
            u[0] = __builtin_amdgcn_mfma_f32_16x16x4f32(ck.a[i][2 * hh + 0], ck.b[2 * i + hh], u[0], 0, 0, 0);
            u[1] = __builtin_amdgcn_mfma_f32_16x16x4f32(ck.a[i][2 * hh + 1], ck.b[2 * i + hh], u[1], 0, 0, 0);
        }
}

template <int K>
struct G1PipeXY {
    static __device__ __forceinline__ void run(f32x4 (&u)[2], G1Chunk& cur, const f32x4* T, const float* buf, int i0, int j, int kq)
    {
        G1Chunk nxt;
        __builtin_amdgcn_sched_barrier(0);
        if (K + 1 < 8) g1_load_xy<(K + 1 < 8 ? K + 1 : 0)>(nxt, T, buf, i0, j, kq);
        g1_mfma_xy(u, cur);
        if (K + 1 < 8) {
#pragma unroll
            for (int g = 0; g < 12; ++g) {
                __builtin_amdgcn_sched_group_barrier(0x008, 1, 0);
                __builtin_amdgcn_sched_group_barrier(0x100, 1, 0);
            }
            __builtin_amdgcn_sched_group_barrier(0x008, 4, 0);
        }
        __builtin_amdgcn_sched_barrier(0);
        if (K + 1 < 8) G1PipeXY<K + 1>::run(u, nxt, T, buf, i0, j, kq);
    }
};
template <>
struct G1PipeXY<8> {
    static __device__ __forceinline__ void run(f32x4 (&)[2], G1Chunk&, const f32x4*, const float*, int, int, int) {}
};

__device__ __forceinline__ int team_quarter_at(int step) { return (0x2130 >> (4 * step)) & 3; }

__device__ __forceinline__ void team_tile_gemm(f32x4 (&u)[2], const float* table, const float* bufs, int member, int lane)
{
    const int n = lane & 15, kq = lane >> 4;
    const int i0 = n >> 3, j = n & 7;
    const f32x4* T = reinterpret_cast<const f32x4*>(table) + lane;
    const int zoff = (kq >> 1) * 128 + qoff(kq & 1, 2 * member + i0, j);
    u[0] = f32x4{0.f, 0.f, 0.f, 0.f};
    u[1] = f32x4{0.f, 0.f, 0.f, 0.f};
    TeamZ zc;
    team_z_load(zc, T, bufs, 0, zoff);
#pragma unroll 1
    for (int s = 0; s < 4; ++s) {
        const int Q = team_quarter_at(s);
        TeamZ zn;
        team_z_load(zn, T, bufs, team_quarter_at(s < 3 ? s + 1 : 3), zoff);
        if (Q == member) {
            const float* buf = bufs + member * kQuarterFloats;
            G1Chunk first;
            g1_load_xy<0>(first, T, buf, i0, j, kq);
            G1PipeXY<0>::run(u, first, T, buf, i0, j, kq);
        }
        __builtin_amdgcn_sched_barrier(0);
        team_z_mfma(u, zc);
        __builtin_amdgcn_sched_barrier(0);
        zc = zn;
    }
}

struct TeamAcc {
    f32x4 xy[2];
    f32x4 z[2][4];
};

template <int K>
__device__ __forceinline__ void g1_load_team(G1Chunk& ck, const f32x4* T, const f32x4* Tz, const float* buf, int i0, int j, int kq)
{
    if (K < 8) {
        const int c0 = 4 * (K & 3);
#pragma unroll
        for (int i = 0; i < 4; ++i) {
            const int c = c0 + i;
            ck.a[i] = T[((K < 4 ? 0 : 16) + c) * 64];
#pragma unroll
            for (int hh = 0; hh < 2; ++hh)
                ck.b[2 * i + hh] = (K < 4) ? buf[c * 128 + qoff(i0, j, 4 * hh + kq)]
                                           : buf[c * 128 + qoff(i0, 4 * hh + kq, j)];
        }
    } else {
        const int cpp = K - 8;
        ck.a[0] = Tz[cpp * 64];
#pragma unroll
        for (int ci = 0; ci < 2; ++ci)
#pragma unroll
            for (int t = 0; t < 4; ++t)
                ck.b[4 * ci + t] = buf[(2 * (2 * cpp + ci) + (kq >> 1)) * 128 + qoff(kq & 1, 2 * t + i0, j)];
    }
}

template <int K>
__device__ __forceinline__ void g1_mfma_team(TeamAcc& a, const G1Chunk& ck)
{
    if (K < 8) {
#pragma unroll
        for (int i = 0; i < 4; ++i)
#pragma unroll
            for (int hh = 0; hh < 2; ++hh) {
                a.xy[0] = __builtin_amdgcn_mfma_f32_16x16x4f32(ck.a[i][2 * hh + 0], ck.b[2 * i + hh], a.xy[0], 0, 0, 0);
                a.xy[1] = __builtin_amdgcn_mfma_f32_16x16x4f32(ck.a[i][2 * hh + 1], ck.b[2 * i + hh], a.xy[1], 0, 0, 0);
            }
    } else {
#pragma unroll
        for (int ci = 0; ci < 2; ++ci)
#pragma unroll
            for (int t = 0; t < 4; ++t) {
                a.z[0][t] = __builtin_amdgcn_mfma_f32_16x16x4f32(ck.a[0][2 * ci + 0], ck.b[4 * ci + t], a.z[0][t], 0, 0, 0);
                a.z[1][t] = __builtin_amdgcn_mfma_f32_16x16x4f32(ck.a[0][2 * ci + 1], ck.b[4 * ci + t], a.z[1][t], 0, 0, 0);
            }
    }
}

template <int K>
struct G1PipeTeam {
    static __device__ __forceinline__ void run(TeamAcc& a, G1Chunk& cur, const f32x4* T, const f32x4* Tz, const float* buf,
                                               int i0, int j, int kq)
    {
        G1Chunk nxt;
        if (K + 1 < 12) g1_load_team<K + 1>(nxt, T, Tz, buf, i0, j, kq);
        __builtin_amdgcn_sched_barrier(0);
        g1_mfma_team<K>(a, cur);
        __builtin_amdgcn_sched_barrier(0);
        if (K + 1 < 12) G1PipeTeam<K + 1>::run(a, nxt, T, Tz, buf, i0, j, kq);
    }
};
template <>
struct G1PipeTeam<12> {
    static __device__ __forceinline__ void run(TeamAcc&, G1Chunk&, const f32x4*, const f32x4*, const float*, int, int, int) {}
};

__device__ __forceinline__ void gemm1_quarter_team(TeamAcc& a, const float* table, const float* buf, int lane, int Q)
{
    const int n = lane & 15, kq = lane >> 4;
    const int i0 = n >> 3, j = n & 7;
    const f32x4* T = reinterpret_cast<const f32x4*>(table) + lane;
    const f32x4* Tz = T + (32 + 4 * Q) * 64;
#pragma unroll
    for (int m = 0; m < 2; ++m) {
        a.xy[m] = f32x4{0.f, 0.f, 0.f, 0.f};
#pragma unroll
        for (int t = 0; t < 4; ++t) a.z[m][t] = f32x4{0.f, 0.f, 0.f, 0.f};
    }
    G1Chunk first;
    g1_load_team<0>(first, T, Tz, buf, i0, j, kq);
    G1PipeTeam<0>::run(a, first, T, Tz, buf, i0, j, kq);
}

struct TgtRegs {
    float2 q[16];
};

template <bool TGT>
__device__ __forceinline__ void tgt_regs_load(TgtRegs& r, const float* __restrict__ tgt, int b, int tid)
{
    if (TGT) {
        if (tid >= 256) {
            const float* V = tgt + (long)b * (16 * 512) + ((tid >> 6) & 3) * 128 + 2 * (tid & 63);
#pragma unroll
            for (int c = 0; c < 16; ++c) r.q[c] = *reinterpret_cast<const float2*>(V + c * 512);
        } else {
#pragma unroll
            for (int c = 0; c < 16; ++c) r.q[c] = float2{0.0f, 0.0f};
        }
    } else {
        const float* ft = tgt + (long)b * (32 * 64);
        const int l = tid & 63, t = tid >> 7, m2 = (tid >> 6) & 1;
#pragma unroll
        for (int k = 0; k < 2; ++k)
            r.q[k] = float2{ft[(16 * m2 + 4 * (l >> 4) + 2 * k) * 64 + 16 * t + (l & 15)],
                            ft[(16 * m2 + 4 * (l >> 4) + 2 * k + 1) * 64 + 16 * t + (l & 15)]};
    }
}

template <bool TGT>
__device__ __forceinline__ void tgt_regs_store(float* srcT, float* buf, const TgtRegs& r, int tid)
{
    if (TGT) {
        if (tid >= 256) {
            const int i = 2 * (tid & 63), o = qoff(i >> 6, (i >> 3) & 7, i & 7);
#pragma unroll
            for (int c = 0; c < 16; ++c) *reinterpret_cast<float2*>(buf + c * 128 + o) = r.q[c];
        }
    } else {
        *reinterpret_cast<f32x4*>(srcT + tid * kSrcStride + 16) = f32x4{r.q[0].x, r.q[0].y, r.q[1].x, r.q[1].y};
    }
}

__device__ __forceinline__ void team_round(f32x4 (&u)[2], const float* table, float* bufs, TeamSync& ts, int team, int member,
                                           unsigned rounds_before, int lane)
{
    team_signal(&ts.arrive[team], lane);
    team_wait(&ts.arrive[team], 4u * (rounds_before + 1u));
    team_tile_gemm(u, table, bufs, member, lane);
    team_signal(&ts.done[team], lane);
}

__device__ __forceinline__ void team_head(f32x4 (&v)[2], const f32x4 (&u)[2], const DualFrags& f)
{
    v[0] = f.bias[0];
    v[1] = f.bias[1];
#pragma unroll
    for (int m = 0; m < 2; ++m) {
        const f32x4 x = relu4(u[m]);
#pragma unroll
        for (int r = 0; r < 4; ++r) {
            v[0] = __builtin_amdgcn_mfma_f32_16x16x4f32(f.a2[m][r][0], x[r], v[0], 0, 0, 0);
            v[1] = __builtin_amdgcn_mfma_f32_16x16x4f32(f.a2[m][r][1], x[r], v[1], 0, 0, 0);
        }
    }
}

__device__ __forceinline__ float team_sumsq(const f32x4 (&v)[2])
{
    float ss = 0.0f;
#pragma unroll
    for (int m2 = 0; m2 < 2; ++m2)
#pragma unroll
        for (int r = 0; r < 4; ++r) ss = fmaf(v[m2][r], v[m2][r], ss);
    ss += __shfl_xor(ss, 16, 64);
    ss += __shfl_xor(ss, 32, 64);
    return ss;
}

}
```

### 3dahv_amd/ops.py

```python
from __future__ import annotations

import collections
import contextvars
import math

import torch

from . import _lib

_VOL = (16, 8, 8, 8)


_SPLIT_F16 = contextvars.ContextVar("ahv_split_f16", default=False)


class split_f16_scorer:

    def __init__(self, enabled: bool = True):
        self.enabled = bool(enabled)
        self._token = None

    def __enter__(self):
        self._token = _SPLIT_F16.set(self.enabled)
        return self

    def __exit__(self, *exc):
        _SPLIT_F16.reset(self._token)
        return False


def _stream(dev=None) -> int:
    return torch.cuda.current_stream(dev).cuda_stream


def _call(dev: torch.device, name: str, *args) -> None:
    lib = _lib.load()
    if dev.type != "cuda":
        raise RuntimeError("3dahv_amd ops run on the GPU only (no CPU fallback); got a tensor on %s" % dev)
    with torch.cuda.device(dev):
        _lib.check(getattr(lib, name)(*args, torch.cuda.current_stream(dev).cuda_stream), name)


def _need_gpu(*tensors: torch.Tensor) -> torch.device:
    dev = tensors[0].device
    for t in tensors:
        if not t.is_cuda:
            raise RuntimeError(
                "3dahv_amd ops run on the GPU only (no CPU fallback); got a tensor on %s" % t.device)
        if t.device != dev:
            raise RuntimeError("Expected all tensors to be on the same device, found %s and %s" % (dev, t.device))
        if t.dtype != torch.float32:
            raise RuntimeError("expected float32 tensors (the reference path is fp32), got %s" % t.dtype)
    return dev


def _refuse_grad(name: str, *tensors: torch.Tensor) -> None:
    if torch.is_grad_enabled() and any(t is not None and t.requires_grad for t in tensors):
        raise RuntimeError("%s has no autograd edge: call it under torch.no_grad() / on detached tensors, or use "
                           "score_hypotheses_autograd / rotate_volume / forward_3d2d, which are differentiable" % name)


def _head(W1: torch.Tensor, W2: torch.Tensor, b2: torch.Tensor):
    if W1.numel() != 32 * 384 or W2.numel() != 32 * 32 or b2.numel() != 32:
        raise RuntimeError("head weights must be (32,384[,1,1]), (32,32[,1,1]), (32,)")
    return W1.detach().reshape(32, 384).contiguous(), W2.detach().reshape(32, 32).contiguous(), b2.detach().contiguous()


def rotate_volume(volume: torch.Tensor, rotation_matrix: torch.Tensor, padding_mode: str = "zeros") -> torch.Tensor:
    if torch.is_grad_enabled():
        if rotation_matrix.requires_grad:
            raise NotImplementedError("rotate_volume: no gradient w.r.t. rotation_matrix is implemented for the op-level "
                                      "rotation (32 KB materialised per hypothesis); detach it, or score with "
                                      "score_hypotheses, whose autograd edge carries d score / d R")
        if volume.requires_grad:
            return _RotateVolumeFn.apply(volume, rotation_matrix)
    return _rotate_volume_nograd(volume, rotation_matrix, padding_mode)


@torch.no_grad()
def _rotate_volume_nograd(volume: torch.Tensor, rotation_matrix: torch.Tensor, padding_mode: str = "zeros") -> torch.Tensor:
    if padding_mode != "zeros":
        raise NotImplementedError("only padding_mode='zeros' (the only mode the reference uses) is implemented")
    if volume.dim() != 5:
        raise RuntimeError("volume must be 5-D (N,C,D,H,W), got %s" % (tuple(volume.shape),))
    if rotation_matrix.dim() != 3 or tuple(rotation_matrix.shape[1:]) != (3, 3):
        raise RuntimeError("rotation_matrix must be (N,3,3), got %s" % (tuple(rotation_matrix.shape),))
    N, C, D, H, W = volume.shape
    if rotation_matrix.shape[0] != N:
        raise RuntimeError("Expected volume and rotation_matrix to have the same batch size, got %d and %d"
                           % (N, rotation_matrix.shape[0]))
    _need_gpu(volume, rotation_matrix)
    volume = volume.detach()
    if N > 1 and volume.stride(0) == 0 and volume[0].is_contiguous():
        src, stride = volume[0], 0
    else:
        src = volume.contiguous()
        stride = C * D * H * W
    R = rotation_matrix.detach().contiguous()
    out = torch.empty((N, C, D, H, W), dtype=torch.float32, device=volume.device)
    _call(out.device, "ahv_rotate_volume_f32", src.data_ptr(), stride, R.data_ptr(), N, C, D, H, W, out.data_ptr())
    return out


def forward_3d2d(img_feat: torch.Tensor, W1: torch.Tensor, W2: torch.Tensor, b2: torch.Tensor) -> torch.Tensor:
    if torch.is_grad_enabled() and any(t.requires_grad for t in (img_feat, W1, W2, b2)):
        return _Forward3d2dFn.apply(img_feat, W1, W2, b2)
    return _forward_3d2d_nograd(img_feat, W1, W2, b2)


@torch.no_grad()
def _forward_3d2d_nograd(img_feat: torch.Tensor, W1: torch.Tensor, W2: torch.Tensor, b2: torch.Tensor) -> torch.Tensor:
    if img_feat.dim() != 5 or tuple(img_feat.shape[1:]) != _VOL:
        raise RuntimeError("img_feat must be (M,16,8,8,8), got %s" % (tuple(img_feat.shape),))
    _need_gpu(img_feat, W1, W2, b2)
    W1, W2, b2 = _head(W1, W2, b2)
    x = img_feat.detach().contiguous()
    M = x.shape[0]
    out = torch.empty((M, 32, 64), dtype=torch.float32, device=x.device)
    _call(out.device, "ahv_forward_3d2d_f32", x.data_ptr(), W1.data_ptr(), W2.data_ptr(), b2.data_ptr(), M,
          out.data_ptr())
    return out


def score_features(f_src: torch.Tensor, f_tgt: torch.Tensor) -> torch.Tensor:
    _refuse_grad("score_features", f_src, f_tgt)
    if f_src.dim() != 4 or tuple(f_src.shape[2:]) != (32, 64) or tuple(f_tgt.shape) != (f_src.shape[0], 32, 64):
        raise RuntimeError("expected f_src (B,N,32,64) and f_tgt (B,32,64)")
    _need_gpu(f_src, f_tgt)
    B, N = f_src.shape[:2]
    a, t = f_src.detach().contiguous(), f_tgt.detach().contiguous()
    out = torch.empty((B, N), dtype=torch.float32, device=a.device)
    _call(out.device, "ahv_score_features_f32", a.data_ptr(), t.data_ptr(), B, N, out.data_ptr())
    return out


@torch.no_grad()
def unpack_best(best_key: torch.Tensor):
    B = best_key.numel()
    score = torch.empty((B,), dtype=torch.float32, device=best_key.device)
    idx = torch.empty((B,), dtype=torch.int64, device=best_key.device)
    _call(best_key.device, "ahv_unpack_best", best_key.data_ptr(), B, score.data_ptr(), idx.data_ptr())
    return score, idx


@torch.no_grad()
def argmax(scores: torch.Tensor, n_offset: int = 0, return_key: bool = False):
    if scores.dim() != 2:
        raise RuntimeError("scores must be (B,N)")
    _need_gpu(scores)
    B, N = scores.shape
    if N == 0:
        raise RuntimeError("max(): Expected reduction dim 1 to have non-zero size.")
    s = scores.detach().contiguous()
    key = torch.empty((B,), dtype=torch.int64, device=s.device)
    _call(key.device, "ahv_argmax_f32", s.data_ptr(), B, N, n_offset, key.data_ptr(), _lib.AHV_SCORE_RESET_BEST)
    if return_key:
        return key
    return unpack_best(key)


def score_hypotheses(vol_src: torch.Tensor, feat_tgt: torch.Tensor, R: torch.Tensor, W1: torch.Tensor,
                     W2: torch.Tensor, b2: torch.Tensor, n_offset: int = 0, want_scores: bool = True,
                     best_key: torch.Tensor | None = None, reset_best: bool | None = None,
                     split_f16: bool | None = None, clock_stamps: torch.Tensor | None = None,
                     no_teams: bool = False, spare_cus: int = 0):
    if (want_scores and clock_stamps is None and torch.is_grad_enabled()
            and any(t.requires_grad for t in (vol_src, feat_tgt, R, W1, W2, b2))):
        return _ScoreFn.apply(vol_src, feat_tgt, R, W1, W2, b2, n_offset, best_key, reset_best, split_f16)
    with torch.no_grad():
        return _score_hypotheses_nograd(vol_src, feat_tgt, R, W1, W2, b2, n_offset, want_scores, best_key, reset_best,
                                        split_f16, clock_stamps, no_teams=no_teams, spare_cus=spare_cus)


def score_plan(B: int, N: int, no_teams: bool = False, split_f16: bool = False, spare_cus: int = 0):
    import ctypes
    flags = ((_lib.AHV_SCORE_NO_TEAMS if no_teams else 0) | (_lib.AHV_SCORE_SPLIT_F16 if split_f16 else 0) |
             (int(spare_cus) << _lib.AHV_SCORE_SPARE_CUS_SHIFT))
    gx, gy, n_main = ctypes.c_int(), ctypes.c_int(), ctypes.c_int64()
    _lib.check(_lib.load().ahv_diag_score_plan(B, N, flags, ctypes.byref(gx), ctypes.byref(gy), ctypes.byref(n_main)),
               "ahv_diag_score_plan")
    return gx.value, gy.value, n_main.value


def verify_pair(vol_src: torch.Tensor, vol_tgt: torch.Tensor, R: torch.Tensor, W1: torch.Tensor, W2: torch.Tensor,
                b2: torch.Tensor, n_offset: int = 0, want_scores: bool = True, best_key: torch.Tensor | None = None,
                reset_best: bool | None = None, split_f16: bool | None = None, want_feat_tgt: bool = False,
                clock_stamps: torch.Tensor | None = None, no_teams: bool = False, spare_cus: int = 0):
    _refuse_grad("verify_pair", vol_src, vol_tgt, R, W1, W2, b2)
    if vol_tgt.dim() != 5 or tuple(vol_tgt.shape) != tuple(vol_src.shape):
        raise RuntimeError("vol_tgt must have vol_src's shape (B,16,8,8,8), got %s" % (tuple(vol_tgt.shape),))
    split = bool(_SPLIT_F16.get() if split_f16 is None else split_f16)
    with torch.no_grad():
        feat = None
        if want_feat_tgt or split:
            feat = torch.empty((vol_src.shape[0], 32, 64), dtype=torch.float32, device=vol_src.device)
        scores, key = _score_hypotheses_nograd(vol_src, vol_tgt, R, W1, W2, b2, n_offset, want_scores, best_key, reset_best,
                                               split, clock_stamps, no_teams=no_teams, spare_cus=spare_cus,
                                               tgt_is_volume=True, feat_tgt_out=feat)
    return (scores, key, feat) if want_feat_tgt else (scores, key)


def _score_hypotheses_nograd(vol_src, feat_tgt, R, W1, W2, b2, n_offset, want_scores, best_key, reset_best, split_f16,
                             clock_stamps, no_teams=False, spare_cus=0, tgt_is_volume=False, feat_tgt_out=None):
    if vol_src.dim() != 5 or tuple(vol_src.shape[1:]) != _VOL:
        raise RuntimeError("vol_src must be (B,16,8,8,8), got %s" % (tuple(vol_src.shape),))
    B = vol_src.shape[0]
    if not tgt_is_volume and tuple(feat_tgt.shape) != (B, 32, 64):
        raise RuntimeError("feat_tgt must be (B,32,64), got %s" % (tuple(feat_tgt.shape),))
    if R.dim() == 3 and tuple(R.shape[1:]) == (3, 3):
        N, rstride = R.shape[0], 0
    elif R.dim() == 4 and R.shape[0] == B and tuple(R.shape[2:]) == (3, 3):
        N, rstride = R.shape[1], R.shape[1] * 9
    else:
        raise RuntimeError("R must be (N,3,3) or (B,N,3,3), got %s" % (tuple(R.shape),))
    dev = _need_gpu(vol_src, feat_tgt, R, W1, W2, b2)
    W1, W2, b2 = _head(W1, W2, b2)
    vs, ft, Rc = vol_src.detach().contiguous(), feat_tgt.detach().contiguous(), R.detach().contiguous()
    scores = torch.empty((B, N), dtype=torch.float32, device=dev) if want_scores else None
    if best_key is None:
        best_key = torch.empty((B,), dtype=torch.int64, device=dev)
        reset_best = True
    elif best_key.dtype != torch.int64 or best_key.numel() != B or not best_key.is_cuda:
        raise RuntimeError("best_key must be a GPU int64 tensor of B elements")
    flags = _lib.AHV_SCORE_RESET_BEST if reset_best else 0
    if _SPLIT_F16.get() if split_f16 is None else split_f16:
        flags |= _lib.AHV_SCORE_SPLIT_F16
    if no_teams:
        flags |= _lib.AHV_SCORE_NO_TEAMS
    if not 0 <= int(spare_cus) <= 255:
        raise RuntimeError("spare_cus must be in 0..255")
    flags |= int(spare_cus) << _lib.AHV_SCORE_SPARE_CUS_SHIFT
    lib = _lib.load()
    head = (vs.data_ptr(), ft.data_ptr(), Rc.data_ptr(), rstride, n_offset, W1.data_ptr(), W2.data_ptr(), b2.data_ptr(),
            B, N, scores.data_ptr() if scores is not None else None, best_key.data_ptr())
    if clock_stamps is not None and (clock_stamps.dtype != torch.int64 or clock_stamps.device != dev or
                                     clock_stamps.numel() < 4 * lib.ahv_device_cu_count()):
        raise RuntimeError("clock_stamps must be an int64 tensor of 4 * CU-count elements on %s" % dev)
    with torch.cuda.device(dev):
        if tgt_is_volume:
            _lib.check(lib.ahv_verify_pair_f32(*head, feat_tgt_out.data_ptr() if feat_tgt_out is not None else None, flags,
                                               clock_stamps.data_ptr() if clock_stamps is not None else None,
                                               _stream(dev)), "ahv_verify_pair_f32")
        elif clock_stamps is None:
            _lib.check(lib.ahv_score_hypotheses_f32(*head, flags, _stream(dev)), "ahv_score_hypotheses_f32")
        else:
            _lib.check(lib.ahv_score_hypotheses_clocked_f32(*head, flags, clock_stamps.data_ptr(), _stream(dev)),
                       "ahv_score_hypotheses_clocked_f32")
    return scores, best_key


@torch.no_grad()
def score_hypotheses_train(vol_src: torch.Tensor, feat_tgt: torch.Tensor, R: torch.Tensor, W1: torch.Tensor, W2: torch.Tensor,
                           b2: torch.Tensor):
    if vol_src.dim() != 5 or tuple(vol_src.shape[1:]) != _VOL:
        raise RuntimeError("vol_src must be (B,16,8,8,8), got %s" % (tuple(vol_src.shape),))
    B = vol_src.shape[0]
    if tuple(feat_tgt.shape) != (B, 32, 64):
        raise RuntimeError("feat_tgt must be (B,32,64), got %s" % (tuple(feat_tgt.shape),))
    N, rstride = _rot_layout(R, B)
    dev = _need_gpu(vol_src, feat_tgt, R, W1, W2, b2)
    W1c, W2c, b2c = _head(W1, W2, b2)
    vs, ft, Rc = (t.detach().contiguous() for t in (vol_src, feat_tgt, R))
    lib = _lib.load()
    nbytes = lib.ahv_score_hypotheses_backward_workspace_bytes(B, N)
    ws = torch.empty((max(nbytes, 16) // 4,), dtype=torch.float32, device=dev)
    scores = torch.empty((B, N), dtype=torch.float32, device=dev)
    _call(dev, "ahv_score_hypotheses_train_f32", vs.data_ptr(), ft.data_ptr(), Rc.data_ptr(), rstride, W1c.data_ptr(),
          W2c.data_ptr(), b2c.data_ptr(), B, N, scores.data_ptr(), ws.data_ptr(), ws.numel() * 4)
    return scores, ws


@torch.no_grad()
def score_hypotheses_backward(vol_src: torch.Tensor, feat_tgt: torch.Tensor, R: torch.Tensor, W1: torch.Tensor,
                              W2: torch.Tensor, b2: torch.Tensor, grad_scores: torch.Tensor, workspace: torch.Tensor | None = None):
    if vol_src.dim() != 5 or tuple(vol_src.shape[1:]) != _VOL:
        raise RuntimeError("vol_src must be (B,16,8,8,8), got %s" % (tuple(vol_src.shape),))
    B = vol_src.shape[0]
    if tuple(feat_tgt.shape) != (B, 32, 64):
        raise RuntimeError("feat_tgt must be (B,32,64), got %s" % (tuple(feat_tgt.shape),))
    N, rstride = _rot_layout(R, B)
    if tuple(grad_scores.shape) != (B, N):
        raise RuntimeError("grad_scores must be (B,N) = %s, got %s" % ((B, N), tuple(grad_scores.shape)))
    dev = _need_gpu(vol_src, feat_tgt, R, W1, W2, b2, grad_scores)
    W1c, W2c, b2c = _head(W1, W2, b2)
    vs, ft, Rc, gs = (t.detach().contiguous() for t in (vol_src, feat_tgt, R, grad_scores))
    lib = _lib.load()
    nbytes = lib.ahv_score_hypotheses_backward_workspace_bytes(B, N)
    saved = workspace is not None
    if saved:
        if workspace.device != dev or workspace.dtype != torch.float32 or workspace.numel() * 4 < nbytes:
            raise RuntimeError("workspace is not the one score_hypotheses_train returned for these shapes")
        ws = workspace
    else:
        ws = torch.empty((max(nbytes, 16) // 4,), dtype=torch.float32, device=dev)
    g_vol = torch.empty((B,) + _VOL, dtype=torch.float32, device=dev)
    g_ft = torch.empty((B, 32, 64), dtype=torch.float32, device=dev)
    g_W1 = torch.empty((32, 384), dtype=torch.float32, device=dev)
    g_W2 = torch.empty((32, 32), dtype=torch.float32, device=dev)
    g_b2 = torch.empty((32,), dtype=torch.float32, device=dev)
    _call(dev, "ahv_score_hypotheses_backward_saved_f32" if saved else "ahv_score_hypotheses_backward_f32", vs.data_ptr(),
          ft.data_ptr(), Rc.data_ptr(), rstride,
          W1c.data_ptr(), W2c.data_ptr(), b2c.data_ptr(), B, N, gs.data_ptr(), ws.data_ptr(), ws.numel() * 4,
          g_vol.data_ptr(), g_ft.data_ptr(), g_W1.data_ptr(), g_W2.data_ptr(), g_b2.data_ptr())
    return g_vol, g_ft, g_W1, g_W2, g_b2


class _RotateVolumeFn(torch.autograd.Function):

    @staticmethod
    def forward(ctx, volume, rotation_matrix):
        out = _rotate_volume_nograd(volume, rotation_matrix)
        N = volume.shape[0]
        ctx.shared = bool(N > 1 and volume.stride(0) == 0 and volume[0].is_contiguous())
        ctx.vshape = tuple(volume.shape)
        ctx.save_for_backward(rotation_matrix.detach().contiguous())
        return out

    @staticmethod
    def backward(ctx, grad_out):
        (R,) = ctx.saved_tensors
        N, C, D, H, W = ctx.vshape
        g = grad_out.contiguous()
        dev = g.device
        if ctx.shared:
            gv = torch.empty((1, C, D, H, W), dtype=torch.float32, device=dev)
            _call(dev, "ahv_rotate_volume_backward_f32", g.data_ptr(), 0, R.data_ptr(), N, C, D, H, W, gv.data_ptr())
            full = torch.zeros((N, C, D, H, W), dtype=torch.float32, device=dev)
            full[0] = gv[0]
            return full, None
        gv = torch.empty((N, C, D, H, W), dtype=torch.float32, device=dev)
        _call(dev, "ahv_rotate_volume_backward_f32", g.data_ptr(), C * D * H * W, R.data_ptr(), N, C, D, H, W,
              gv.data_ptr())
        return gv, None


class _ScoreFn(torch.autograd.Function):

    @staticmethod
    def forward(ctx, vol_src, feat_tgt, R, W1, W2, b2, n_offset=0, best_key=None, reset_best=None, split_f16=None, need_key=True):
        ctx.ws = None
        plain = n_offset == 0 and best_key is None and not split_f16 and (split_f16 is not None or not _SPLIT_F16.get())
        plain = plain and any(ctx.needs_input_grad[i] for i in (0, 1, 3, 4, 5))
        if plain:
            scores, ctx.ws = score_hypotheses_train(vol_src, feat_tgt, R, W1, W2, b2)
            if need_key:
                key = argmax(scores, return_key=True)
            else:
                key = torch.full((vol_src.shape[0],), _lib.AHV_KEY_EMPTY, dtype=torch.int64, device=scores.device)
        else:
            scores, key = _score_hypotheses_nograd(vol_src, feat_tgt, R, W1, W2, b2, n_offset, True, best_key, reset_best,
                                                   split_f16, None)
        ctx.save_for_backward(vol_src, feat_tgt, R, W1, W2, b2)
        ctx.mark_non_differentiable(key)
        return scores, key

    @staticmethod
    def backward(ctx, grad_scores, _grad_key):
        vol_src, feat_tgt, R, W1, W2, b2 = ctx.saved_tensors
        ws, ctx.ws = ctx.ws, None
        gs = grad_scores.contiguous()
        need = ctx.needs_input_grad
        g_R = None
        if need[2]:
            g_R = score_rotation_grad(vol_src, feat_tgt, R, W1, W2, b2, gs)
            if R.dim() == 3:
                g_R = g_R.sum(dim=0)
        if not (need[0] or need[1] or need[3] or need[4] or need[5]):
            return (None, None, g_R) + (None,) * 8
        g_vol, g_ft, g_W1, g_W2, g_b2 = score_hypotheses_backward(vol_src, feat_tgt, R, W1, W2, b2, gs, workspace=ws)
        return (g_vol, g_ft, g_R, g_W1.reshape(W1.shape), g_W2.reshape(W2.shape), g_b2.reshape(b2.shape),
                None, None, None, None, None)


def score_hypotheses_autograd(vol_src, feat_tgt, R, W1, W2, b2) -> torch.Tensor:
    return _ScoreFn.apply(vol_src, feat_tgt, R, W1, W2, b2, 0, None, None, None, False)[0]


class _Forward3d2dFn(torch.autograd.Function):

    @staticmethod
    def forward(ctx, vol, W1, W2, b2):
        ctx.save_for_backward(vol, W1, W2, b2)
        return _forward_3d2d_nograd(vol, W1, W2, b2)

    @staticmethod
    def backward(ctx, dF):
        vol, W1, W2, b2 = ctx.saved_tensors
        M = vol.shape[0]
        eye = torch.eye(3, dtype=torch.float32, device=vol.device).reshape(1, 3, 3)
        gs = torch.full((M, 1), 64.0, dtype=torch.float32, device=vol.device)
        g_vol, _, g_W1, g_W2, g_b2 = score_hypotheses_backward(vol, dF.contiguous(), eye, W1, W2, b2, gs)
        return g_vol, g_W1.reshape(W1.shape), g_W2.reshape(W2.shape), g_b2.reshape(b2.shape)


def forward_3d2d_autograd(img_feat, W1, W2, b2) -> torch.Tensor:
    return _Forward3d2dFn.apply(img_feat, W1, W2, b2)


def _rot_layout(R: torch.Tensor, B: int):
    if R.dim() == 3 and tuple(R.shape[1:]) == (3, 3):
        return R.shape[0], 0
    if R.dim() == 4 and R.shape[0] == B and tuple(R.shape[2:]) == (3, 3):
        return R.shape[1], R.shape[1] * 9
    raise RuntimeError("R must be (N,3,3) or (B,N,3,3), got %s" % (tuple(R.shape),))


@torch.no_grad()
def reset_best(best_key: torch.Tensor) -> torch.Tensor:
    if best_key.dtype != torch.int64 or not best_key.is_cuda:
        raise RuntimeError("best_key must be a GPU int64 tensor")
    _call(best_key.device, "ahv_reset_best", best_key.data_ptr(), best_key.numel())
    return best_key


@torch.no_grad()
def select_rotation(best_key: torch.Tensor, R: torch.Tensor, n_offset: int = 0, reset_key: bool = False):
    B = best_key.numel()
    _need_gpu(R)
    N, rstride = _rot_layout(R, B)
    Rc = R.detach().contiguous()
    dev = Rc.device
    score = torch.empty((B,), dtype=torch.float32, device=dev)
    idx = torch.empty((B,), dtype=torch.int64, device=dev)
    R_out = torch.empty((B, 3, 3), dtype=torch.float32, device=dev)
    _call(dev, "ahv_select_rotation_f32", best_key.data_ptr(), Rc.data_ptr(), rstride, n_offset, N, B,
          R_out.data_ptr(), score.data_ptr(), idx.data_ptr(), _lib.AHV_SELECT_RESET_KEY if reset_key else 0)
    return score, idx, R_out


@torch.no_grad()
def compose_rotations(best_key: torch.Tensor, R: torch.Tensor, D: torch.Tensor, n_offset: int = 0,
                      out: torch.Tensor | None = None) -> torch.Tensor:
    B = best_key.numel()
    _need_gpu(R, D)
    N, rstride = _rot_layout(R, B)
    if D.dim() != 3 or tuple(D.shape[1:]) != (3, 3):
        raise RuntimeError("D must be (N2,3,3)")
    N2 = D.shape[0]
    Rc, Dc = R.detach().contiguous(), D.detach().contiguous()
    if out is None:
        out = torch.empty((B, N2, 3, 3), dtype=torch.float32, device=Rc.device)
    _call(out.device, "ahv_compose_rotations_f32", best_key.data_ptr(), Rc.data_ptr(), rstride, n_offset, N,
          Dc.data_ptr(), N2, B, out.data_ptr())
    return out



_TOPK_WS = {}


def _workspace(cache: dict, key: tuple, nbytes: int, dtype: torch.dtype, given: torch.Tensor | None = None):
    dev = key[0]
    ws = given
    if ws is None and nbytes:
        ws = cache.get(key)
        if ws is None:
            ws = cache[key] = torch.empty((nbytes // dtype.itemsize,), dtype=dtype, device=dev)
    have = 0
    if ws is not None:
        if ws.device != dev or not ws.is_contiguous():
            raise RuntimeError("workspace must be a contiguous tensor on %s" % dev)
        have = ws.numel() * ws.element_size()
    return ws, have


def _topk_k(k) -> int:
    k = int(k)
    if not 1 <= k <= _lib.AHV_TOPK_MAX_K:
        raise RuntimeError("K = %d outside 1..%d" % (k, _lib.AHV_TOPK_MAX_K))
    return k


def _topk_list(keys: torch.Tensor, what: str = "keys"):
    if keys.dim() != 2 or keys.dtype != torch.int64:
        raise RuntimeError("%s must be a (B,K) int64 tensor" % what)
    if not keys.is_cuda:
        raise RuntimeError("3dahv_amd ops run on the GPU only (no CPU fallback); got a tensor on %s" % keys.device)
    if not keys.is_contiguous():
        raise RuntimeError("%s must be contiguous" % what)
    return keys.shape[0], _topk_k(keys.shape[1])


@torch.no_grad()
def topk(scores: torch.Tensor, k: int, n_offset: int = 0, keys: torch.Tensor | None = None, reset: bool | None = None):
    if scores.dim() != 2:
        raise RuntimeError("scores must be (B,N)")
    k = _topk_k(k)
    dev = _need_gpu(scores)
    B, N = scores.shape
    if keys is None:
        keys = torch.empty((B, k), dtype=torch.int64, device=dev)
        reset = True
    elif _topk_list(keys) != (B, k) or keys.device != dev:
        raise RuntimeError("keys must be a (B,K) = %s int64 tensor on %s" % ((B, k), dev))
    s = scores.detach().contiguous()
    ws, have = _workspace(_TOPK_WS, (dev, B, N, k), _lib.load().ahv_topk_workspace_bytes(B, N, k), torch.int64)
    _call(dev, "ahv_topk_f32", s.data_ptr(), B, N, n_offset, k, keys.data_ptr(), ws.data_ptr() if ws is not None else None,
          have, _lib.AHV_TOPK_RESET_LIST if reset else 0)
    return keys


@torch.no_grad()
def merge_topk(lists: torch.Tensor, keys: torch.Tensor | None = None, reset: bool | None = None):
    if lists.dim() != 3 or lists.dtype != torch.int64:
        raise RuntimeError("lists must be a (P,B,K) int64 tensor")
    if not lists.is_cuda:
        raise RuntimeError("3dahv_amd ops run on the GPU only (no CPU fallback); got a tensor on %s" % lists.device)
    P, B, k = lists.shape
    k = _topk_k(k)
    if keys is None:
        keys = torch.empty((B, k), dtype=torch.int64, device=lists.device)
        reset = True
    elif _topk_list(keys) != (B, k) or keys.device != lists.device:
        raise RuntimeError("keys must be a (B,K) = %s int64 tensor on %s" % ((B, k), lists.device))
    ls = lists.contiguous()
    _call(ls.device, "ahv_topk_merge_keys", ls.data_ptr(), P, B, k, keys.data_ptr(), _lib.AHV_TOPK_RESET_LIST if reset else 0)
    return keys


@torch.no_grad()
def select_topk(keys: torch.Tensor, R: torch.Tensor, n_offset: int = 0, reset_keys: bool = False):
    B, k = _topk_list(keys)
    _need_gpu(R)
    if R.device != keys.device:
        raise RuntimeError("Expected all tensors to be on the same device, found %s and %s" % (keys.device, R.device))
    N, rstride = _rot_layout(R, B)
    Rc = R.detach().contiguous()
    dev = Rc.device
    score = torch.empty((B, k), dtype=torch.float32, device=dev)
    idx = torch.empty((B, k), dtype=torch.int64, device=dev)
    R_out = torch.empty((B, k, 3, 3), dtype=torch.float32, device=dev)
    _call(dev, "ahv_select_topk_f32", keys.data_ptr(), k, Rc.data_ptr(), rstride, n_offset, N, B, R_out.data_ptr(),
          score.data_ptr(), idx.data_ptr(), _lib.AHV_SELECT_RESET_KEY if reset_keys else 0)
    return score, idx, R_out


@torch.no_grad()
def compose_rotations_topk(keys: torch.Tensor, R: torch.Tensor, D: torch.Tensor, n_offset: int = 0,
                           out: torch.Tensor | None = None) -> torch.Tensor:
    B, k = _topk_list(keys)
    _need_gpu(R, D)
    if R.device != keys.device:
# ... 552 lines not shown
```

### include/ahv.h

```cpp
#ifndef AHV_H
#define AHV_H

#include <stddef.h>
#include <stdint.h>

#ifdef __cplusplus
extern "C" {
#endif

#define AHV_OK 0
#define AHV_EINVAL (-1)
#define AHV_ELAUNCH (-2)
#define AHV_EDEVICE (-3)

#define AHV_CV 16
#define AHV_S 8
#define AHV_K 384
#define AHV_O 32
#define AHV_P 64
#define AHV_VOL_ELEMS (AHV_CV * AHV_S * AHV_S * AHV_S)
#define AHV_FEAT_ELEMS (AHV_O * AHV_P)

#define AHV_KEY_EMPTY INT64_MIN

#define AHV_SCORE_RESET_BEST 1u
#define AHV_SCORE_SPLIT_F16 2u

#define AHV_SCORE_NO_TEAMS 4u

#define AHV_SELECT_RESET_KEY 1u

int ahv_abi_version(void);

const char* ahv_last_error(void);

int ahv_device_cu_count(void);

int ahv_score_hypotheses_f32(const float* vol_src, const float* feat_tgt, const float* R,
                             int64_t r_batch_stride, int64_t n_offset, const float* W1,
                             const float* W2, const float* b2, int B, int64_t N, float* scores,
                             int64_t* best_key, unsigned flags, void* stream);

int ahv_verify_pair_f32(const float* vol_src, const float* vol_tgt, const float* R, int64_t r_batch_stride,
                        int64_t n_offset, const float* W1, const float* W2, const float* b2, int B, int64_t N,
                        float* scores, int64_t* best_key, float* feat_tgt_out, unsigned flags, uint64_t* clock_stamps,
                        void* stream);

int ahv_unpack_best(const int64_t* best_key, int B, float* best_score, int64_t* best_idx, void* stream);

int ahv_reset_best(int64_t* best_key, int B, void* stream);

int ahv_rotate_volume_f32(const float* vol, int64_t vol_batch_stride, const float* R, int64_t N,
                          int C, int D, int H, int W, float* out, void* stream);

int ahv_rotate_volume_backward_f32(const float* grad_out, int64_t vol_batch_stride, const float* R, int64_t N,
                                   int C, int D, int H, int W, float* grad_vol, void* stream);

int ahv_forward_3d2d_f32(const float* vol, const float* W1, const float* W2, const float* b2,
                         int64_t M, float* out, void* stream);

int ahv_score_features_f32(const float* f_src, const float* f_tgt, int B, int64_t N, float* scores,
                           void* stream);

int ahv_argmax_f32(const float* scores, int B, int64_t N, int64_t n_offset, int64_t* best_key,
                   unsigned flags, void* stream);

int ahv_select_rotation_f32(int64_t* best_key, const float* R, int64_t r_batch_stride, int64_t n_offset,
                            int64_t N, int B, float* R_out, float* best_score, int64_t* best_idx, unsigned flags,
                            void* stream);

int ahv_coarse_to_fine_f32(const float* vol_src, const float* vol_tgt, const float* R, int64_t r_batch_stride, int64_t N,
                           const float* D, int64_t N2, const float* W1, const float* W2, const float* b2, int B,
                           float* scores_coarse, float* scores_fine, int64_t* keys, uint32_t* sync, float* feat_tgt_out,
                           float* R_pred, float* fine_score, int64_t* fine_idx, float* coarse_score, int64_t* coarse_idx,
                           unsigned flags, void* stream);

int ahv_compose_rotations_f32(const int64_t* best_key, const float* R, int64_t r_batch_stride, int64_t n_offset,
                              int64_t N, const float* D, int64_t N2, int B, float* out, void* stream);

#define AHV_TOPK_MAX_K 64
#define AHV_TOPK_RESET_LIST 1u

size_t ahv_topk_workspace_bytes(int B, int64_t N, int K);

int ahv_topk_f32(const float* scores, int B, int64_t N, int64_t n_offset, int K, int64_t* keys, void* workspace,
                 size_t workspace_bytes, unsigned flags, void* stream);

int ahv_topk_merge_keys(const int64_t* lists, int P, int B, int K, int64_t* keys, unsigned flags, void* stream);

int ahv_select_topk_f32(int64_t* keys, int K, const float* R, int64_t r_batch_stride, int64_t n_offset, int64_t N, int B,
                        float* R_out, float* scores_out, int64_t* idx_out, unsigned flags, void* stream);

int ahv_compose_rotations_topk_f32(const int64_t* keys, int K, const float* R, int64_t r_batch_stride, int64_t n_offset,
                                   int64_t N, const float* D, int64_t N2, int B, float* out, void* stream);

size_t ahv_topk_modes_workspace_bytes(int B, int64_t N, int K);
int ahv_topk_modes_f32(const float* scores, const float* R, int64_t r_batch_stride, int B, int64_t N, int64_t n_offset, int K,
                       float min_trace, int64_t* keys, void* workspace, size_t workspace_bytes, void* stream);

#define AHV_POSTERIOR_MAX_MODES 16
#define AHV_POSTERIOR_RESET_STATE 1u

size_t ahv_pose_posterior_state_bytes(int B, int K);
size_t ahv_pose_posterior_workspace_bytes(int B, int64_t N, int K);
int ahv_pose_posterior_f32(const float* scores, const float* R, int64_t r_batch_stride, int B, int64_t N, const float* anchors,
                           int K, float min_trace, float beta, void* state, void* workspace, size_t workspace_bytes,
                           unsigned flags, void* stream);
int ahv_pose_posterior_merge(const void* states, int P, int B, int K, float beta, void* state, unsigned flags, void* stream);
int ahv_pose_posterior_finish_f32(const void* state, int B, int K, float beta, float* log_z, float* entropy, float* mean_score,
                                  int64_t* n_excluded, float* mode_prob, float* rest_prob, float* mode_R_mean, float* R_mean,
                                  float* mode_spread_deg, float* spread_deg, void* stream);

#define AHV_VIEWS_MAX 16
#define AHV_VIEWS_RESET_BEST 1u
#define AHV_VIEWS_NO_ANGLE_LIMIT 2u

int ahv_view_rotations_f32(const float* Q, int64_t q_batch_stride, const float* A, int B, int V, int64_t N, float* out,
                           void* stream);
int ahv_fuse_view_scores_f32(const float* scores, const float* Q, int64_t q_batch_stride, const float* A, const float* weights,
                             int B, int V, int64_t N, int64_t n_offset, float min_trace, float* fused, int64_t* best_key,
                             unsigned flags, void* stream);

int ahv_random_rotations_f32(uint64_t seed, uint64_t offset, int64_t N, float* out, void* stream);

int ahv_so3_grid_f32(int64_t n_total, int64_t offset, int64_t N, float* out, void* stream);

typedef struct ahv_block_weights {
    const float* w_qkv;
    const float* w_out;
    const float* b_out;
    const float* ln1_g;
    const float* ln1_b;
    const float* w_ff1;
    const float* b_ff1;
    const float* w_ff2;
    const float* b_ff2;
    const float* ln2_g;
    const float* ln2_b;
} ahv_block_weights;

size_t ahv_transformer_workspace_bytes(int B);

int ahv_transformer_blocks_f32(const ahv_block_weights* blocks, int depth, float* x_src, float* x_tgt, int B,
                               void* workspace, size_t workspace_bytes, void* stream);

typedef struct ahv_aligner_weights {
    const float* w_emb;
    const float* w_conv1;
    const float* w_conv2;
    const float* posemb;
    const float* gn_g;
    const float* gn_b;
    const float* w_in[2];
    const float* b_in[2];
    const float* w_out[2];
    const float* b_out[2];
    const float* w3d_1;
    const float* w3d_2;
    const ahv_block_weights* blocks;
    int depth;
} ahv_aligner_weights;

size_t ahv_forward_2d3d_workspace_bytes(int B);

int ahv_forward_2d3d_f32(const ahv_aligner_weights* w, const float* layer4_src, const float* layer4_tgt, int B,
                         void* workspace, size_t workspace_bytes, float* vol_src, float* vol_tgt, void* stream);

size_t ahv_score_hypotheses_backward_workspace_bytes(int B, int64_t N);

int ahv_score_hypotheses_backward_f32(const float* vol_src, const float* feat_tgt, const float* R,
                                      int64_t r_batch_stride, const float* W1, const float* W2, const float* b2,
                                      int B, int64_t N, const float* grad_scores, void* workspace,
                                      size_t workspace_bytes, float* grad_vol_src, float* grad_feat_tgt,
                                      float* grad_W1, float* grad_W2, float* grad_b2, void* stream);

int ahv_score_hypotheses_train_f32(const float* vol_src, const float* feat_tgt, const float* R, int64_t r_batch_stride,
                                   const float* W1, const float* W2, const float* b2, int B, int64_t N, float* scores,
                                   void* workspace, size_t workspace_bytes, void* stream);

int ahv_score_hypotheses_backward_saved_f32(const float* vol_src, const float* feat_tgt, const float* R,
                                            int64_t r_batch_stride, const float* W1, const float* W2, const float* b2,
                                            int B, int64_t N, const float* grad_scores, void* workspace,
                                            size_t workspace_bytes, float* grad_vol_src, float* grad_feat_tgt,
                                            float* grad_W1, float* grad_W2, float* grad_b2, void* stream);

size_t ahv_score_rotation_grad_workspace_bytes(int B, int64_t N);

int ahv_score_rotation_grad_f32(const float* vol_src, const float* feat_tgt, const float* R, int64_t r_batch_stride,
                                const float* W1, const float* W2, const float* b2, int B, int64_t N,
                                const float* grad_scores, void* workspace, size_t workspace_bytes, float* grad_R,
                                void* stream);

#define AHV_SO3_MAX_LADDER 8

int ahv_so3_ascent_candidates_f32(const float* R_cur, const float* grad_R, const float* theta, const float* ladder, int L,
                                  int B, int K, float* R_cand, void* stream);

int ahv_so3_ascent_select_f32(const float* R_cand, const float* cand_scores, const float* ladder, int L, int B, int K,
                              float* R_cur, float* score_cur, float* theta, void* stream);

#ifdef __cplusplus
}
#endif
#endif
```

### include/ahv_diag.h

```cpp
#ifndef AHV_DIAG_H
#define AHV_DIAG_H

#include "ahv.h"

#ifdef __cplusplus
extern "C" {
#endif

#define AHV_SCORE_SPARE_CUS_SHIFT 8
#define AHV_SCORE_SPARE_CUS_MASK 0xFF00u
#define AHV_SCORE_SPARE_CUS(k) (((unsigned)(k) << AHV_SCORE_SPARE_CUS_SHIFT) & AHV_SCORE_SPARE_CUS_MASK)

int ahv_score_hypotheses_clocked_f32(const float* vol_src, const float* feat_tgt, const float* R,
                                     int64_t r_batch_stride, int64_t n_offset, const float* W1,
                                     const float* W2, const float* b2, int B, int64_t N, float* scores,
                                     int64_t* best_key, unsigned flags, uint64_t* clock_stamps, void* stream);

int ahv_diag_score_plan(int B, int64_t N, unsigned flags, int* gx, int* gy, int64_t* n_main);

#ifdef __cplusplus
}
#endif
#endif
```

Before: 73.34 million hypotheses/s.

## Share target features across verify blocks via global workspace instead of recomputing

In the fp32 verify-pair kernel, block 0 now publishes the normalised target feature rows to a persistent global workspace with atomic counters. Deferring blocks skip loading and encoding the target volume and copy the published features into LDS, falling back to building them late if they are not ready. This aims to remove the duplicated per-block target-head computation, at the cost of cross-block spin and atomic coordination plus a cached device workspace.

```diff
diff --git a/3dahv_amd/_lib.py b/3dahv_amd/_lib.py
--- a/3dahv_amd/_lib.py
+++ b/3dahv_amd/_lib.py
@@ -12,6 +12,8 @@
 AHV_SCORE_SPLIT_F16 = 2
 AHV_SCORE_NO_TEAMS = 4
 AHV_SCORE_SPARE_CUS_SHIFT = 8
+AHV_VERIFY_NO_SHARE = 0x10000
+AHV_VERIFY_NO_PUBLISH = 0x20000
 AHV_SELECT_RESET_KEY = 1
 AHV_KEY_EMPTY = -(1 << 63)
 AHV_TOPK_MAX_K = 64
@@ -36,6 +38,8 @@
     "ahv_score_hypotheses_clocked_f32": (_int, [_vp, _vp, _vp, _i64, _i64, _vp, _vp, _vp, _int, _i64, _vp, _vp, _u32,
                                                 _vp, _vp]),
     "ahv_verify_pair_f32": (_int, [_vp, _vp, _vp, _i64, _i64, _vp, _vp, _vp, _int, _i64, _vp, _vp, _vp, _u32, _vp, _vp]),
+    "ahv_verify_pair_workspace_bytes": (ctypes.c_size_t, [_int]),
+    "ahv_verify_pair_ws_f32": (_int, [_vp, _vp, _vp, _i64, _i64, _vp, _vp, _vp, _int, _i64, _vp, _vp, _vp, _u32, _vp, _vp, _vp]),
     "ahv_unpack_best": (_int, [_vp, _int, _vp, _vp, _vp]),
     "ahv_reset_best": (_int, [_vp, _int, _vp]),
     "ahv_rotate_volume_f32": (_int, [_vp, _i64, _vp, _i64, _int, _int, _int, _int, _vp, _vp]),
diff --git a/3dahv_amd/csrc/ahv_abi.hip b/3dahv_amd/csrc/ahv_abi.hip
--- a/3dahv_amd/csrc/ahv_abi.hip
+++ b/3dahv_amd/csrc/ahv_abi.hip
@@ -116,7 +116,7 @@
 static int score_common(const char* who, const float* vol_src, const float* tgt, bool tgt_is_volume, const float* R,
                         int64_t r_batch_stride, int64_t n_offset, const float* W1, const float* W2, const float* b2, int B,
                         int64_t N, float* scores, int64_t* best_key, float* feat_tgt_out, unsigned flags,
-                        uint64_t* clock_stamps, void* stream)
+                        uint64_t* clock_stamps, void* stream, void* workspace = nullptr, unsigned extra_flags = 0u)
 {
     if (B < 0 || N < 0) return fail(AHV_EINVAL, "%s: negative size (B=%d, N=%lld)", who, B, (long long)N);
     if (B > 0 && N > 0 && (!vol_src || !tgt || !R || !W1 || !W2 || !b2))
@@ -125,7 +125,7 @@
         return fail(AHV_EINVAL, "%s: r_batch_stride %lld must be 0 or >= N*9", who, (long long)r_batch_stride);
     if (n_offset < 0 || n_offset + N > 4294967296ll)
         return fail(AHV_EINVAL, "%s: n_offset + N must fit in 32 bits", who);
-    if (flags & ~(AHV_SCORE_RESET_BEST | AHV_SCORE_SPLIT_F16 | AHV_SCORE_NO_TEAMS | AHV_SCORE_SPARE_CUS_MASK))
+    if (flags & ~(AHV_SCORE_RESET_BEST | AHV_SCORE_SPLIT_F16 | AHV_SCORE_NO_TEAMS | AHV_SCORE_SPARE_CUS_MASK | extra_flags))
         return fail(AHV_EINVAL, "%s: unknown flags 0x%x", who, flags);
     const bool split = (flags & AHV_SCORE_SPLIT_F16) != 0;
     hipStream_t s = static_cast<hipStream_t>(stream);
@@ -154,6 +154,9 @@
     a.scores = scores; a.best_key = best_key; a.feat_tgt_out = feat_tgt_out; a.num_cu = cu;
     a.spare_cu = (int)((flags & AHV_SCORE_SPARE_CUS_MASK) >> AHV_SCORE_SPARE_CUS_SHIFT);
     a.split_f16 = split; a.no_teams = (flags & AHV_SCORE_NO_TEAMS) != 0; a.clock_stamps = clock_stamps;
+    a.workspace = workspace;
+    a.verify_no_share = (flags & AHV_VERIFY_NO_SHARE) != 0;
+    a.verify_no_publish = (flags & AHV_VERIFY_NO_PUBLISH) != 0;
     hipError_t e = ahv::launch_score_hypotheses(a, s);
     if (e != hipSuccess) return hip_fail("score: launch", e);
     return AHV_OK;
@@ -198,6 +201,19 @@
 {
     return score_common("verify_pair", vol_src, vol_tgt, true, R, r_batch_stride, n_offset, W1, W2, b2, B, N, scores,
                         best_key, feat_tgt_out, flags, clock_stamps, stream);
+}
+
+size_t ahv_verify_pair_workspace_bytes(int B) { return B > 0 ? (size_t)B * (32 * 64 + 8) * 4 : 0; }
+
+int ahv_verify_pair_ws_f32(const float* vol_src, const float* vol_tgt, const float* R, int64_t r_batch_stride,
+                           int64_t n_offset, const float* W1, const float* W2, const float* b2, int B, int64_t N,
+                           float* scores, int64_t* best_key, float* feat_tgt_out, unsigned flags, uint64_t* clock_stamps,
+                           void* workspace, void* stream)
+{
+    if (B > 0 && !workspace) return fail(AHV_EINVAL, "verify_pair_ws: null workspace");
+    if (reinterpret_cast<uintptr_t>(workspace) & 15u) return fail(AHV_EINVAL, "verify_pair_ws: workspace must be 16-byte aligned");
+    return score_common("verify_pair_ws", vol_src, vol_tgt, true, R, r_batch_stride, n_offset, W1, W2, b2, B, N, scores,
+                        best_key, feat_tgt_out, flags, clock_stamps, stream, workspace, AHV_VERIFY_NO_SHARE | AHV_VERIFY_NO_PUBLISH);
 }
 
 int ahv_unpack_best(const int64_t* best_key, int B, float* best_score, int64_t* best_idx, void* stream)
diff --git a/3dahv_amd/csrc/ahv_launch.h b/3dahv_amd/csrc/ahv_launch.h
--- a/3dahv_amd/csrc/ahv_launch.h
+++ b/3dahv_amd/csrc/ahv_launch.h
@@ -20,6 +20,9 @@
     bool split_f16;
     bool no_teams;
     uint64_t* clock_stamps;
+    void* workspace = nullptr;
+    bool verify_no_share = false;
+    bool verify_no_publish = false;
 };
 
 struct ScorePlan {
diff --git a/3dahv_amd/csrc/ahv_score.hip b/3dahv_amd/csrc/ahv_score.hip
--- a/3dahv_amd/csrc/ahv_score.hip
+++ b/3dahv_amd/csrc/ahv_score.hip
@@ -180,13 +180,107 @@
     return best;
 }
 
-template <bool SPLIT, bool TGT, bool C2F, bool SAVE_U = false>
+constexpr int kWsFeatWords = 32 * 64, kWsWords = kWsFeatWords + 8;
+constexpr unsigned kVerifyNoShare = 1u, kVerifyNoPublish = 2u;
+
+struct TgtShare {
+    unsigned c0;
+    unsigned s0;
+    unsigned state;
+};
+
+__device__ __forceinline__ void team_tgt_rows(f32x4 (&x)[2], float* lds_src, const float* lds_w1, float* bufs1, TeamSync& ts,
+                                              const NonFinite& nf, const DualFrags& f0, bool nf_w, unsigned gen, int member,
+                                              unsigned rounds_before, int lane)
+{
+    f32x4 u[2], v[2];
+    team_round(u, lds_w1, bufs1, ts, 1, member, rounds_before, lane);
+    if (nf_w || (unsigned)__builtin_amdgcn_readfirstlane((int)nf.tgt_gen) == gen) team_head_exact(v, u, f0);
+    else team_head(v, u, f0);
+    const float inv = 1.0f / fmaxf(sqrtf(team_sumsq(v)), 1e-12f);
+#pragma unroll
+    for (int m2 = 0; m2 < 2; ++m2) {
+        x[m2] = v[m2] * inv;
+        *reinterpret_cast<f32x4*>(lds_src + ((2 * member + m2) * 64 + lane) * kSrcStride + 16) = x[m2];
+    }
+}
+
+#define AHV_LDS_PTR(T) __attribute__((address_space(3))) T*
+__device__ __attribute__((noinline)) void tgt_build_late(const float* vol_tgt, unsigned* ws, int b, AHV_LDS_PTR(float) src3,
+                                                         AHV_LDS_PTR(float) w13, AHV_LDS_PTR(float) q3, AHV_LDS_PTR(TeamSync) ts3,
+                                                         AHV_LDS_PTR(NonFinite) nf3, const float* W2, const float* b2,
+                                                         bool nf_w, unsigned gen, int member, unsigned rounds_before, int lane)
+{
+    float* lds_src = (float*)src3;
+    const float* lds_w1 = (const float*)w13;
+    float* bufs1 = (float*)q3 + 4 * kQuarterFloats;
+    TeamSync* ts = (TeamSync*)ts3;
+    NonFinite* nf = (NonFinite*)nf3;
+    const float* vol_tgt_b = vol_tgt + (long)b * (16 * 512);
+    unsigned* ws_b = ws + (long)b * kWsWords;
+    TgtRegs tv;
+    tgt_regs_load<true>(tv, vol_tgt_b, 0, 256 + member * 64 + lane);
+    bool tbad = false;
+#pragma unroll
+    for (int c = 0; c < 16; ++c) tbad = tbad || non_finite(tv.q[c].x) || non_finite(tv.q[c].y);
+    if (tbad) nf->tgt_gen = gen;
+    tgt_regs_store<true>(lds_src, bufs1 + member * kQuarterFloats, tv, 256 + member * 64 + lane);
+    DualFrags f0;
+    load_dual_frags(f0, W2, b2, lane);
+    f32x4 x[2];
+    team_tgt_rows(x, lds_src, lds_w1, bufs1, *ts, *nf, f0, nf_w, gen, member, rounds_before, lane);
+    team_signal(&ts->tgt_ready, lane);
+    if (member == 0 && lane == 0) {
+        __hip_atomic_fetch_add(ws_b + kWsFeatWords + 2, 1u, __ATOMIC_RELAXED, __HIP_MEMORY_SCOPE_AGENT);
+        __hip_atomic_fetch_add(ws_b + kWsFeatWords + 4, 1u, __ATOMIC_RELAXED, __HIP_MEMORY_SCOPE_AGENT);
+    }
+    team_wait(&ts->done[1], 4u * (rounds_before + 1u));
+}
+
+__device__ __forceinline__ unsigned tgt_decide(TgtShare& sh, TeamSync& ts, float* lds_src, unsigned* ws_b, unsigned gen, bool never, int lane)
+{
+    unsigned prev = 0;
+    if (lane == 0) prev = __hip_atomic_fetch_max(&sh.state, 4u * gen, __ATOMIC_RELAXED, __HIP_MEMORY_SCOPE_WORKGROUP);
+    prev = (unsigned)__builtin_amdgcn_readfirstlane((int)prev);
+    if ((int)(prev - 4u * gen) < 0) {
+        const unsigned c0 = (unsigned)__builtin_amdgcn_readfirstlane((int)__hip_atomic_load(&sh.c0, __ATOMIC_RELAXED, __HIP_MEMORY_SCOPE_WORKGROUP));
+        const unsigned c = (unsigned)__builtin_amdgcn_readfirstlane(
+            (int)__hip_atomic_load(ws_b + kWsFeatWords, __ATOMIC_RELAXED, __HIP_MEMORY_SCOPE_AGENT));
+        unsigned st = 2u;
+        if (c != c0 && !never) {
+            __builtin_amdgcn_fence(__ATOMIC_ACQUIRE, "agent");
+            const f32x4* wf = reinterpret_cast<const f32x4*>(ws_b) + opaque(lane);
+            f32x4 x[8];
+#pragma unroll
+            for (int k = 0; k < 8; ++k) x[k] = wf[k * 64];
+#pragma unroll
+            for (int k = 0; k < 8; ++k) *reinterpret_cast<f32x4*>(lds_src + (k * 64 + lane) * kSrcStride + 16) = x[k];
+            __builtin_amdgcn_s_waitcnt(0xc07f);
+            asm volatile("" ::: "memory");
+            if (lane == 0) {
+                __hip_atomic_fetch_add(&ts.tgt_ready, 4u, __ATOMIC_RELAXED, __HIP_MEMORY_SCOPE_WORKGROUP);
+                __hip_atomic_fetch_add(ws_b + kWsFeatWords + 1, 1u, __ATOMIC_RELAXED, __HIP_MEMORY_SCOPE_AGENT);
+            }
+            st = 1u;
+        }
+        if (lane == 0) __hip_atomic_store(&sh.state, 4u * gen + st, __ATOMIC_RELAXED, __HIP_MEMORY_SCOPE_WORKGROUP);
+        return st;
+    }
+    unsigned s;
+    while ((s = __hip_atomic_load(&sh.state, __ATOMIC_RELAXED, __HIP_MEMORY_SCOPE_WORKGROUP)) == 4u * gen) __builtin_amdgcn_s_sleep(1);
+    asm volatile("" ::: "memory");
+    return (unsigned)__builtin_amdgcn_readfirstlane((int)s) & 3u;
+}
+
+template <bool SPLIT, bool TGT, bool C2F, bool SAVE_U = false, bool SHARE = false>
 __device__ __forceinline__ void score_hypotheses_body(
     const float* __restrict__ vol_src, const float* __restrict__ tgt, const float* __restrict__ R,
     long r_batch_stride, long n_offset, const float* __restrict__ W1, const float* __restrict__ W2,
     const float* __restrict__ b2, int B, long N, long n_main, float* __restrict__ scores,
-    key_t* __restrict__ best_key, float* __restrict__ feat_tgt_out, unsigned long long* __restrict__ clk, const C2fArgs& cf)
-{
+    key_t* __restrict__ best_key, float* __restrict__ feat_tgt_out, unsigned long long* __restrict__ clk, const C2fArgs& cf,
+    unsigned* ws = nullptr, unsigned vflags = 0u)
+{
+    static_assert(!SHARE || (TGT && !SPLIT && !C2F), "the shared target features belong to the fp32 verify instance");
     static_assert(!(SPLIT && TGT), "the split-f16 kernel takes ready-made target features");
     static_assert(!C2F || (TGT && !SPLIT), "the two-stage launch is the fp32 verify kernel");
     static_assert(!SAVE_U || (!SPLIT && !TGT && !C2F), "u is saved by the fp32 scorer with ready-made target features");
@@ -196,6 +290,7 @@
     __shared__ __attribute__((aligned(16))) float lds_q[8 * kQuarterFloats];
     __shared__ TeamSync lds_team;
     __shared__ NonFinite lds_nf;
+    __shared__ TgtShare lds_share;
     __shared__ unsigned long long lds_t_entry[2];
     if (clk != nullptr && threadIdx.x == 0) {
         lds_t_entry[0] = __builtin_amdgcn_s_memrealtime();
@@ -215,6 +310,16 @@
 #endif
     if (!SPLIT && tid < (int)(sizeof(TeamSync) / 4)) reinterpret_cast<unsigned*>(&lds_team)[tid] = 0u;
     if (tid < (int)(sizeof(NonFinite) / 4)) reinterpret_cast<unsigned*>(&lds_nf)[tid] = 0u;
+    bool share = false, defer = false;
+#ifndef AHV_DIAG_NO_EXACT
+    if constexpr (SHARE) {
+        share = ws != nullptr && !(vflags & kVerifyNoShare) && N - n_main < (long)gridDim.x;
+        defer = share && blockIdx.x != 0 && !(n_main + xcd_residue(blockIdx.x, gridDim.x, gridDim.y) < N);
+        if (tid < 3) reinterpret_cast<unsigned*>(&lds_share)[tid] = 0u;
+        if (share && blockIdx.x == 0 && tid == 0)
+            __hip_atomic_fetch_add(ws + (long)blockIdx.y * kWsWords + kWsFeatWords + 3, 1u, __ATOMIC_RELAXED, __HIP_MEMORY_SCOPE_AGENT);
+    }
+#endif
     SrcRegs sv;
     TgtRegs tv;
     W1Regs w1r;
@@ -222,7 +327,7 @@
     if (!SPLIT) {
         if (w1_rows) w1_regs_load(w1r, W1, tid);
         src_regs_load(sv, vol_src + (long)blockIdx.y * (16 * 512), tid);
-        tgt_regs_load<TGT>(tv, tgt, (int)blockIdx.y, tid);
+        tgt_regs_load<TGT>(tv, tgt, (int)blockIdx.y, tid, !defer);
     }
     int w1_exp = 0, w2_exp = 0;
     if (SPLIT) {
@@ -297,7 +402,19 @@
                 for (int c = 0; c < 16; ++c) tbad = tbad || non_finite(tv.q[c].x) || non_finite(tv.q[c].y);
                 if (tbad) lds_nf.tgt_gen = gen;
             }
-            tgt_regs_store<TGT>(lds_src, buf, tv, tid_s);
+            if (!defer) tgt_regs_store<TGT>(lds_src, buf, tv, tid_s);
+            if constexpr (SHARE) {
+                if (share && tid_s == 0) {
+                    unsigned* wc = ws + (long)b * kWsWords + kWsFeatWords;
+                    if (blockIdx.x == 0) {
+                        if (samples_done != 0u) __hip_atomic_fetch_add(wc + 3, 1u, __ATOMIC_RELAXED, __HIP_MEMORY_SCOPE_AGENT);
+                    } else if (defer) {
+                        lds_share.s0 = __hip_atomic_load(wc + 3, __ATOMIC_RELAXED, __HIP_MEMORY_SCOPE_AGENT);
+                        asm volatile("s_waitcnt vmcnt(0)" ::: "memory");
+                        lds_share.c0 = __hip_atomic_load(wc, __ATOMIC_RELAXED, __HIP_MEMORY_SCOPE_AGENT);
+                    }
+                }
+            }
         }
         if (SPLIT) {
             const float* ft = tgt + (long)b * (32 * 64);
@@ -321,34 +438,83 @@
             }
         }
         bool tg_ready = !TGT;
+        bool defer_b = false;
+        if constexpr (SHARE) {
+            if (defer) {
+                const unsigned s0 = (unsigned)__builtin_amdgcn_readfirstlane((int)lds_share.s0);
+                const unsigned p0 = (unsigned)__builtin_amdgcn_readfirstlane((int)lds_share.c0);
+                defer_b = s0 == p0 + 1u;
+                if (!defer_b && team == 1) {
+                    const int tl = 256 + member * 64 + lane_s;
+                    TgtRegs tq;
+                    tgt_regs_load<true>(tq, tgt, b, tl);
+                    bool tbad = false;
+#pragma unroll
+                    for (int c = 0; c < 16; ++c) tbad = tbad || non_finite(tq.q[c].x) || non_finite(tq.q[c].y);
+                    if (tbad) lds_nf.tgt_gen = gen;
+                    tgt_regs_store<true>(lds_src, buf, tq, tl);
+                }
+            }
+        }
         if constexpr (TGT) {
-            if (team == 1) {
-                f32x4 u[2], v[2];
-                team_round(u, lds_w1, lds_q + 4 * kQuarterFloats, lds_team, 1, member, team_rounds, lane_s);
+            if (team == 1 && !defer_b) {
+                f32x4 xr[2];
+                team_tgt_rows(xr, lds_src, lds_w1, lds_q + 4 * kQuarterFloats, lds_team, lds_nf, f0, nf_w, gen, member, team_rounds, lane_s);
                 ++team_rounds;
-                if (nf_w || (unsigned)__builtin_amdgcn_readfirstlane((int)lds_nf.tgt_gen) == gen) team_head_exact(v, u, f0);
-                else team_head(v, u, f0);
-                const float inv = 1.0f / fmaxf(sqrtf(team_sumsq(v)), 1e-12f);
+                const bool publish = SHARE && share && blockIdx.x == 0;
 #pragma unroll
                 for (int m2 = 0; m2 < 2; ++m2) {
-                    const f32x4 x = v[m2] * inv;
-                    *reinterpret_cast<f32x4*>(lds_src + ((2 * member + m2) * 64 + lane_s) * kSrcStride + 16) = x;
+                    const f32x4 x = xr[m2];
                     if (feat_tgt_out != nullptr && blockIdx.x == 0) {
                         const int ol = lane_s;
 #pragma unroll
                         for (int r = 0; r < 4; ++r)
                             feat_tgt_out[(long)b * (32 * 64) + (16 * m2 + 4 * (ol >> 4) + r) * 64 + 16 * member + (ol & 15)] = x[r];
                     }
-                }
+                    if constexpr (SHARE) {
+                        if (publish) {
+                            unsigned* wf = ws + (long)b * kWsWords + 4 * ((2 * member + m2) * 64 + lane_s);
+#pragma unroll
+                            for (int r = 0; r < 4; ++r) __hip_atomic_store(wf + r, __float_as_uint(x[r]), __ATOMIC_RELAXED, __HIP_MEMORY_SCOPE_AGENT);
+                        }
+                    }
+                }
+                if constexpr (SHARE)
+                    if (publish) asm volatile("s_waitcnt vmcnt(0)" ::: "memory");
                 team_signal(&lds_team.tgt_ready, lane_s);
+                if constexpr (SHARE) {
+                    if (ws != nullptr && member == 0) {
+                        unsigned* wc = ws + (long)b * kWsWords + kWsFeatWords;
+                        if (publish) {
+                            team_wait(&lds_team.tgt_ready, 4u * gen);
+                            if (lane_s == 0) __hip_atomic_fetch_add(wc, 1u, __ATOMIC_RELEASE, __HIP_MEMORY_SCOPE_AGENT);
+                        }
+                        if (lane_s == 0) __hip_atomic_fetch_add(wc + 2, 1u, __ATOMIC_RELAXED, __HIP_MEMORY_SCOPE_AGENT);
+                    }
+                }
                 team_wait(&lds_team.done[1], 4u * team_rounds);
             }
         }
-        auto tg_wait = [&]() {
+        auto tg_wait = [&]() -> bool {
+            bool redo = false;
             if (TGT && !tg_ready) {
+                if constexpr (SHARE) {
+                    if (defer_b) {
+                        unsigned* ws_b = ws + (long)b * kWsWords;
+                        if (tgt_decide(lds_share, lds_team, lds_src, ws_b, samples_done + 1u, (vflags & kVerifyNoPublish) != 0u, lane) == 2u &&
+                            team == 1) {
+                            tgt_build_late(tgt, ws, b, (AHV_LDS_PTR(float))lds_src, (AHV_LDS_PTR(float))lds_w1, (AHV_LDS_PTR(float))lds_q,
+                                           (AHV_LDS_PTR(TeamSync))&lds_team, (AHV_LDS_PTR(NonFinite))&lds_nf, W2, b2, nf_w,
+                                           samples_done + 1u, member, team_rounds, lane);
+                            ++team_rounds;
+                            redo = true;
+                        }
+                    }
+                }
                 team_wait(&lds_team.tgt_ready, 4u * (samples_done + 1u));
                 tg_ready = true;
             }
+            return redo;
         };
 #ifdef AHV_STAMPS
         wg_t_loop = __builtin_amdgcn_s_memrealtime();
@@ -525,7 +691,11 @@
                 gemm1_quarter_pipe<2>(acc, lds_w1, buf, lane, [] {}); wave_lds_fence(); AHV_TS(8)
             }
 
-            tg_wait();
+            if (tg_wait()) {
+                Rn = Rb[h * 9 + rl];
+                h -= hstep;
+                continue;
+            }
             float s;
             if constexpr (SPLIT) {
                 const Gemm2Scale sc = gemm2_split_scale(acc, exp_sum);
@@ -575,6 +745,8 @@
         }
 #endif
         }
+        if constexpr (SHARE)
+            if (defer_b && team == 1 && residue < N_s) tg_wait();
         if (key_s != nullptr && lane == 0 && best != kKeyEmpty) atomicMax(key_s + b, best);
       }
         ++samples_done;
@@ -582,7 +754,7 @@
             const int bn = b + (int)gridDim.y < B ? b + (int)gridDim.y : b;
             const int tid_e = wave * 64 + opaque(lane);
             src_regs_load(sv, vol_src + (long)bn * (16 * 512), tid_e);
-            tgt_regs_load<TGT>(tv, tgt, bn, tid_e);
+            tgt_regs_load<TGT>(tv, tgt, bn, tid_e, !defer);
         }
         if constexpr (C2F) {
             __syncthreads();
@@ -643,10 +815,11 @@
     const float* __restrict__ vol_src, const float* __restrict__ tgt, const float* __restrict__ R,
     long r_batch_stride, long n_offset, const float* __restrict__ W1, const float* __restrict__ W2,
     const float* __restrict__ b2, int B, long N, long n_main, float* __restrict__ scores,
-    key_t* __restrict__ best_key, float* __restrict__ feat_tgt_out, unsigned long long* __restrict__ clk)
-{
-    score_hypotheses_body<SPLIT, TGT, false>(vol_src, tgt, R, r_batch_stride, n_offset, W1, W2, b2, B, N, n_main, scores, best_key,
-                                             feat_tgt_out, clk, C2fArgs{});
+    key_t* __restrict__ best_key, float* __restrict__ feat_tgt_out, unsigned long long* __restrict__ clk, unsigned* ws,
+    unsigned vflags)
+{
+    score_hypotheses_body<SPLIT, TGT, false, false, TGT && !SPLIT>(vol_src, tgt, R, r_batch_stride, n_offset, W1, W2, b2, B, N, n_main,
+                                                                   scores, best_key, feat_tgt_out, clk, C2fArgs{}, ws, vflags);
 }
 
 __global__ __launch_bounds__(kDualThreads, 2) void score_hypotheses_train_kernel(
@@ -707,19 +880,21 @@
     const dim3 grid(p.gx, p.gy), block(kDualThreads);
     auto* key = reinterpret_cast<key_t*>(a.best_key);
     auto* clk = reinterpret_cast<unsigned long long*>(a.clock_stamps);
+    unsigned* wsp = a.tgt_is_volume && !a.split_f16 ? static_cast<unsigned*>(a.workspace) : nullptr;
+    const unsigned vfl = (a.verify_no_share ? kVerifyNoShare : 0u) | (a.verify_no_publish ? kVerifyNoPublish : 0u);
     if (a.split_f16) {
         if (a.tgt_is_volume) return hipErrorInvalidValue;
         hipLaunchKernelGGL((score_hypotheses_dual_kernel<true, false>), grid, block, 0, stream, a.vol_src, a.tgt, a.R,
                            (long)a.r_batch_stride, (long)a.n_offset, a.W1, a.W2, a.b2, a.B, (long)a.N, (long)p.n_main, a.scores,
-                           key, a.feat_tgt_out, clk);
+                           key, a.feat_tgt_out, clk, wsp, vfl);
     } else if (a.tgt_is_volume) {
         hipLaunchKernelGGL((score_hypotheses_dual_kernel<false, true>), grid, block, 0, stream, a.vol_src, a.tgt, a.R,
                            (long)a.r_batch_stride, (long)a.n_offset, a.W1, a.W2, a.b2, a.B, (long)a.N, (long)p.n_main, a.scores,
-                           key, a.feat_tgt_out, clk);
+                           key, a.feat_tgt_out, clk, wsp, vfl);
     } else {
         hipLaunchKernelGGL((score_hypotheses_dual_kernel<false, false>), grid, block, 0, stream, a.vol_src, a.tgt, a.R,
                            (long)a.r_batch_stride, (long)a.n_offset, a.W1, a.W2, a.b2, a.B, (long)a.N, (long)p.n_main, a.scores,
-                           key, a.feat_tgt_out, clk);
+                           key, a.feat_tgt_out, clk, wsp, vfl);
     }
     return hipGetLastError();
 }
diff --git a/3dahv_amd/csrc/ahv_team.h b/3dahv_amd/csrc/ahv_team.h
--- a/3dahv_amd/csrc/ahv_team.h
+++ b/3dahv_amd/csrc/ahv_team.h
@@ -227,10 +227,10 @@
 };
 
 template <bool TGT>
-__device__ __forceinline__ void tgt_regs_load(TgtRegs& r, const float* __restrict__ tgt, int b, int tid)
+__device__ __forceinline__ void tgt_regs_load(TgtRegs& r, const float* __restrict__ tgt, int b, int tid, bool build = true)
 {
     if (TGT) {
-        if (tid >= 256) {
+        if (tid >= 256 && build) {
             const float* V = tgt + (long)b * (16 * 512) + ((tid >> 6) & 3) * 128 + 2 * (tid & 63);
 #pragma unroll
             for (int c = 0; c < 16; ++c) r.q[c] = *reinterpret_cast<const float2*>(V + c * 512);
diff --git a/3dahv_amd/ops.py b/3dahv_amd/ops.py
--- a/3dahv_amd/ops.py
+++ b/3dahv_amd/ops.py
@@ -185,7 +185,8 @@
 def verify_pair(vol_src: torch.Tensor, vol_tgt: torch.Tensor, R: torch.Tensor, W1: torch.Tensor, W2: torch.Tensor,
                 b2: torch.Tensor, n_offset: int = 0, want_scores: bool = True, best_key: torch.Tensor | None = None,
                 reset_best: bool | None = None, split_f16: bool | None = None, want_feat_tgt: bool = False,
-                clock_stamps: torch.Tensor | None = None, no_teams: bool = False, spare_cus: int = 0):
+                clock_stamps: torch.Tensor | None = None, no_teams: bool = False, spare_cus: int = 0,
+                workspace: torch.Tensor | None = None, share: bool = True, publish: bool = True):
     _refuse_grad("verify_pair", vol_src, vol_tgt, R, W1, W2, b2)
     if vol_tgt.dim() != 5 or tuple(vol_tgt.shape) != tuple(vol_src.shape):
         raise RuntimeError("vol_tgt must have vol_src's shape (B,16,8,8,8), got %s" % (tuple(vol_tgt.shape),))
@@ -194,14 +195,42 @@
         feat = None
         if want_feat_tgt or split:
             feat = torch.empty((vol_src.shape[0], 32, 64), dtype=torch.float32, device=vol_src.device)
+        vflags = (0 if share else _lib.AHV_VERIFY_NO_SHARE) | (0 if publish else _lib.AHV_VERIFY_NO_PUBLISH)
         scores, key = _score_hypotheses_nograd(vol_src, vol_tgt, R, W1, W2, b2, n_offset, want_scores, best_key, reset_best,
                                                split, clock_stamps, no_teams=no_teams, spare_cus=spare_cus,
-                                               tgt_is_volume=True, feat_tgt_out=feat)
+                                               tgt_is_volume=True, feat_tgt_out=feat, workspace=workspace, verify_flags=vflags)
     return (scores, key, feat) if want_feat_tgt else (scores, key)
 
 
+_VERIFY_WS: dict = {}
+_VERIFY_WS_WORDS = 32 * 64 + 8
+
+
+def _verify_ws(dev: torch.device, stream: int, B: int):
+    if stream != 0 and torch.cuda.is_current_stream_capturing():
+        ws = torch.empty(max(B, 1) * _VERIFY_WS_WORDS, dtype=torch.int32, device=dev).fill_(0)
+        return ws, ws.data_ptr()
+    ent = _VERIFY_WS.get((dev.index, stream))
+    if ent is None or ent[2] < B:
+        ws = torch.empty(max(B, 1) * _VERIFY_WS_WORDS, dtype=torch.int32, device=dev).fill_(0)
+        ent = _VERIFY_WS[(dev.index, stream)] = (ws, ws.data_ptr(), B)
+    return ent[0], ent[1]
+
+
+def verify_workspace(device, B: int) -> torch.Tensor:
+    device = torch.device(device)
+    if device.index is None:
+        device = torch.device("cuda", torch.cuda.current_device())
+    return _verify_ws(device, _stream(device), int(B))[0]
+
+
+def verify_workspace_counters(workspace: torch.Tensor, B: int) -> torch.Tensor:
+    return workspace[:B * _VERIFY_WS_WORDS].view(B, _VERIFY_WS_WORDS)[:, 2048:2053].to(torch.int64)
+
+
 def _score_hypotheses_nograd(vol_src, feat_tgt, R, W1, W2, b2, n_offset, want_scores, best_key, reset_best, split_f16,
-                             clock_stamps, no_teams=False, spare_cus=0, tgt_is_volume=False, feat_tgt_out=None):
+                             clock_stamps, no_teams=False, spare_cus=0, tgt_is_volume=False, feat_tgt_out=None,
+                             workspace=None, verify_flags=0):
     if vol_src.dim() != 5 or tuple(vol_src.shape[1:]) != _VOL:
         raise RuntimeError("vol_src must be (B,16,8,8,8), got %s" % (tuple(vol_src.shape),))
     B = vol_src.shape[0]
@@ -236,8 +265,18 @@
     if clock_stamps is not None and (clock_stamps.dtype != torch.int64 or clock_stamps.device != dev or
                                      clock_stamps.numel() < 4 * lib.ahv_device_cu_count()):
         raise RuntimeError("clock_stamps must be an int64 tensor of 4 * CU-count elements on %s" % dev)
+    if workspace is not None and (workspace.dtype != torch.int32 or workspace.device != dev or not workspace.is_contiguous() or
+                                  workspace.numel() < B * _VERIFY_WS_WORDS):
+        raise RuntimeError("workspace must be a contiguous int32 tensor of ahv_verify_pair_workspace_bytes(B) bytes on %s" % dev)
     with torch.cuda.device(dev):
-        if tgt_is_volume:
+        if tgt_is_volume and not flags & _lib.AHV_SCORE_SPLIT_F16:
+            st = _stream(dev)
+            workspace, ws_ptr = (workspace, workspace.data_ptr()) if workspace is not None else _verify_ws(dev, st, B)
+            _lib.check(lib.ahv_verify_pair_ws_f32(*head, feat_tgt_out.data_ptr() if feat_tgt_out is not None else None,
+                                                  flags | verify_flags,
+                                                  clock_stamps.data_ptr() if clock_stamps is not None else None,
+                                                  ws_ptr, st), "ahv_verify_pair_ws_f32")
+        elif tgt_is_volume:
             _lib.check(lib.ahv_verify_pair_f32(*head, feat_tgt_out.data_ptr() if feat_tgt_out is not None else None, flags,
                                                clock_stamps.data_ptr() if clock_stamps is not None else None,
                                                _stream(dev)), "ahv_verify_pair_f32")
diff --git a/include/ahv.h b/include/ahv.h
--- a/include/ahv.h
+++ b/include/ahv.h
@@ -45,6 +45,12 @@
                         int64_t n_offset, const float* W1, const float* W2, const float* b2, int B, int64_t N,
                         float* scores, int64_t* best_key, float* feat_tgt_out, unsigned flags, uint64_t* clock_stamps,
                         void* stream);
+
+size_t ahv_verify_pair_workspace_bytes(int B);
+int ahv_verify_pair_ws_f32(const float* vol_src, const float* vol_tgt, const float* R, int64_t r_batch_stride,
+                           int64_t n_offset, const float* W1, const float* W2, const float* b2, int B, int64_t N,
+                           float* scores, int64_t* best_key, float* feat_tgt_out, unsigned flags, uint64_t* clock_stamps,
+                           void* workspace, void* stream);
 
 int ahv_unpack_best(const int64_t* best_key, int B, float* best_score, int64_t* best_idx, void* stream);
 
diff --git a/include/ahv_diag.h b/include/ahv_diag.h
--- a/include/ahv_diag.h
+++ b/include/ahv_diag.h
@@ -11,6 +11,9 @@
 #define AHV_SCORE_SPARE_CUS_MASK 0xFF00u
 #define AHV_SCORE_SPARE_CUS(k) (((unsigned)(k) << AHV_SCORE_SPARE_CUS_SHIFT) & AHV_SCORE_SPARE_CUS_MASK)
 
+#define AHV_VERIFY_NO_SHARE 0x10000u
+#define AHV_VERIFY_NO_PUBLISH 0x20000u
+
 int ahv_score_hypotheses_clocked_f32(const float* vol_src, const float* feat_tgt, const float* R,
                                      int64_t r_batch_stride, int64_t n_offset, const float* W1,
                                      const float* W2, const float* b2, int B, int64_t N, float* scores,
```

After: 73.35 million hypotheses/s, median of 4. About the same (+0.0%).
